# yamoling/lle

Measured on AMD Instinct MI355X. Metric: env-steps/s (agents x envs x steps/s), level-6 batch 65536, higher is better.
Workload: dtype u8

## Files before the change

lle_amd/csrc/obs_stream.hpp:

```cpp
#pragma once
#include <hip/hip_runtime.h>
#include <stdint.h>

#include <type_traits>

#include "tables.h"

namespace lle {

__device__ __forceinline__ void wave_sync() {
    __builtin_amdgcn_fence(__ATOMIC_RELEASE, "wavefront");
    __builtin_amdgcn_wave_barrier();
    __builtin_amdgcn_fence(__ATOMIC_ACQUIRE, "wavefront");
}

__device__ __forceinline__ uint32_t xcd_block(uint32_t b, uint32_t n_blocks) {
    const uint32_t x = b & 7u, q = n_blocks >> 3, r = n_blocks & 7u;
    return x * q + (x < r ? x : r) + (b >> 3);
}
__device__ __forceinline__ uint32_t xcd_block_dir(uint32_t b, uint32_t n_blocks, uint32_t flags) {
    const uint32_t blk = xcd_block(b, n_blocks);
    return (flags & LAUNCH_REVERSE) ? n_blocks - 1u - blk : blk;
}

__device__ __forceinline__ uint32_t row_rotation(uint32_t wave_id, uint32_t rows_per_wave, int64_t n_here, uint32_t flags) {
    const uint32_t r = wave_id & (rows_per_wave - 1u);
    return ((flags & LAUNCH_ROTATE_ROWS) && (int64_t)r < n_here && n_here == (int64_t)rows_per_wave) ? r : 0u;
}
__device__ __forceinline__ uint32_t rotated(uint32_t k, uint32_t rot, uint32_t n) {
    const uint32_t kk = k + rot;
    return kk >= n ? kk - n : kk;
}

typedef uint32_t u32x4 __attribute__((ext_vector_type(4)));
#define LLE_COPY_ROWS(SRC)                                                                                              \
    for (uint32_t r0 = wave_in_wg; r0 < rows; r0 += 8 * waves_per_wg) {                                                \
        const uint32_t r1 = r0 + waves_per_wg, r2 = r1 + waves_per_wg, r3 = r2 + waves_per_wg, r4 = r3 + waves_per_wg, \
                       r5 = r4 + waves_per_wg, r6 = r5 + waves_per_wg, r7 = r6 + waves_per_wg;                          \
        const u32x4 z = {0, 0, 0, 0};                                                                                   \
        u32x4 v0 = SRC(r0), v1 = z, v2 = z, v3 = z, v4 = z, v5 = z, v6 = z, v7 = z;                                      \
        if (r1 < rows) v1 = SRC(r1);                                                                                    \
        if (r2 < rows) v2 = SRC(r2);                                                                                    \
        if (r3 < rows) v3 = SRC(r3);                                                                                    \
        if (r4 < rows) {                                                                                                \
            v4 = SRC(r4);                                                                                               \
            if (r5 < rows) v5 = SRC(r5);                                                                                \
            if (r6 < rows) v6 = SRC(r6);                                                                                \
            if (r7 < rows) v7 = SRC(r7);                                                                                \
        }                                                                                                               \
        __builtin_amdgcn_sched_barrier(0);                        \
        dst[r0 * 64] = v0;                                                                                              \
        if (r1 < rows) dst[r1 * 64] = v1;                                                                               \
        if (r2 < rows) dst[r2 * 64] = v2;                                                                               \
        if (r3 < rows) dst[r3 * 64] = v3;                                                                               \
        if (r4 < rows) {                                                                                                \
            dst[r4 * 64] = v4;                                                                                          \
            if (r5 < rows) dst[r5 * 64] = v5;                                                                           \
            if (r6 < rows) dst[r6 * 64] = v6;                                                                           \
            if (r7 < rows) dst[r7 * 64] = v7;                                                                           \
        }                                                                                                               \
    }
__device__ __forceinline__ void copy_tables_to_lds(const uint8_t* __restrict__ tables, uint8_t* lds, uint32_t tab_bytes,
                                                   uint32_t lane, uint32_t wave_in_wg, uint32_t waves_per_wg) {
    const u32x4* __restrict__ src = reinterpret_cast<const u32x4*>(tables) + lane;
    u32x4* dst = reinterpret_cast<u32x4*>(lds) + lane;
    const uint32_t rows = tab_bytes / 1024;
#define LLE_SRC1(r) src[(r) * 64]
    LLE_COPY_ROWS(LLE_SRC1)
#undef LLE_SRC1
}

__device__ __forceinline__ void copy_tables2_to_lds(const uint8_t* __restrict__ t1, uint32_t bytes1, const uint8_t* __restrict__ t2, uint32_t bytes2,
                                                    uint8_t* lds, uint32_t lane, uint32_t wave_in_wg, uint32_t waves_per_wg) {
    const u32x4* __restrict__ s1 = reinterpret_cast<const u32x4*>(t1) + lane;
    const u32x4* __restrict__ s2 = reinterpret_cast<const u32x4*>(t2) + lane;
    u32x4* dst = reinterpret_cast<u32x4*>(lds) + lane;
    const uint32_t rows1 = bytes1 / 1024, rows = rows1 + bytes2 / 1024;
#define LLE_SRC2(r) (*((r) < rows1 ? s1 + (r) * 64 : s2 + ((r) - rows1) * 64))
    LLE_COPY_ROWS(LLE_SRC2)
#undef LLE_SRC2
}
#undef LLE_COPY_ROWS

__device__ __forceinline__ void expand_packed_tables(const uint8_t* __restrict__ pk, uint8_t* lds, uint32_t HW, uint32_t n_lay, uint32_t lds_meta, uint32_t lds_dyn,
                                                     uint32_t tail_bytes, uint32_t tid, uint32_t T) {
    const uint64_t* __restrict__ m4 = reinterpret_cast<const uint64_t*>(pk);
    const uint16_t* __restrict__ idx = reinterpret_cast<const uint16_t*>(pk + packed_meta_bytes(HW));
    const uint64_t* __restrict__ lay = reinterpret_cast<const uint64_t*>(pk + packed_meta_bytes(HW) + packed_idx_bytes(n_lay));
    const uint4* __restrict__ tail = reinterpret_cast<const uint4*>(pk + packed_meta_bytes(HW) + packed_idx_bytes(n_lay) + ((n_lay * 8u + 15u) & ~15u));
    const uint32_t n4 = (HW + 3u) / 4u, nt = tail_bytes / 16u;
    const uint64_t w0 = tid < n4 ? m4[tid] : 0ull;
    const uint32_t i0 = tid < n_lay ? (uint32_t)idx[tid] : 0u;
    const uint64_t l0 = tid < n_lay ? lay[tid] : 0ull;
    uint4 t0 = {0u, 0u, 0u, 0u};
    if (tid < nt) t0 = tail[tid];
    auto widen = [](uint64_t w) { return uint4{(uint32_t)w & 0xFFFFu, (uint32_t)(w >> 16) & 0xFFFFu, (uint32_t)(w >> 32) & 0xFFFFu, (uint32_t)(w >> 48)}; };
    uint4* z = reinterpret_cast<uint4*>(lds);
    for (uint32_t i = tid; i < lds_meta / 16u; i += T) z[i] = uint4{0u, 0u, 0u, 0u};
    uint4* md = reinterpret_cast<uint4*>(lds + lds_meta);
    if (tid < n4) md[tid] = widen(w0);
    for (uint32_t i = tid + T; i < n4; i += T) md[i] = widen(m4[i]);
    uint4* td = reinterpret_cast<uint4*>(lds + lds_dyn);
    if (tid < nt) td[tid] = t0;
    for (uint32_t i = tid + T; i < nt; i += T) td[i] = tail[i];
    asm volatile("s_waitcnt lgkmcnt(0)\n\ts_barrier" ::: "memory");
    uint64_t* ld = reinterpret_cast<uint64_t*>(lds);
    if (tid < n_lay) ld[i0] = l0;
    for (uint32_t i = tid + T; i < n_lay; i += T) ld[idx[i]] = lay[i];
}

__device__ __forceinline__ uint32_t mad24(uint32_t a, uint32_t b, uint32_t c) {
    uint32_t r;
    asm("v_mad_u32_u24 %0, %1, %2, %3" : "=v"(r) : "v"(a), "v"(b), "v"(c));
    return r;
}

template <typename T>
__device__ __forceinline__ void small_store(T* p, T v) {
#ifdef LLE_SMALL_WT
    if constexpr (sizeof(T) == 1) {
        asm volatile("global_store_byte %0, %1, off sc1" ::"v"(p), "v"((uint32_t)(uint8_t)v) : "memory");
    } else if constexpr (sizeof(T) == 2) {
        asm volatile("global_store_short %0, %1, off sc1" ::"v"(p), "v"((uint32_t)(uint16_t)v) : "memory");
    } else if constexpr (sizeof(T) == 4) {
        uint32_t w;
        __builtin_memcpy(&w, &v, 4);
        asm volatile("global_store_dword %0, %1, off sc1" ::"v"(p), "v"(w) : "memory");
    } else {
        static_assert(sizeof(T) == 8, "small_store: 1, 2, 4 or 8 bytes");
        uint64_t w;
        __builtin_memcpy(&w, &v, 8);
        asm volatile("global_store_dwordx2 %0, %1, off sc1" ::"v"(p), "v"(w) : "memory");
    }
#else
    *p = v;
#endif
}

template <bool WT>
__device__ __forceinline__ void stream_store(uint4* p, const uint4& v) {
    if constexpr (WT) {
        const u32x4 w = {v.x, v.y, v.z, v.w};
        asm volatile("global_store_dwordx4 %0, %1, off sc1\n\ts_nop 1" ::"v"(p), "v"(w));
    } else {
        *p = v;
    }
}

template <bool WT>
__device__ __forceinline__ void stream_row(uint4* __restrict__ dst, const uint4* srcv, uint32_t first, uint32_t n_chunks, uint32_t lane) {
    uint32_t c = first + lane;
    for (; c + 192u < n_chunks; c += 256u) {
        const uint4 q0 = srcv[c], q1 = srcv[c + 64u], q2 = srcv[c + 128u], q3 = srcv[c + 192u];
        stream_store<WT>(dst + c, q0);
        stream_store<WT>(dst + c + 64u, q1);
        stream_store<WT>(dst + c + 128u, q2);
        stream_store<WT>(dst + c + 192u, q3);
    }
    for (; c < n_chunks; c += 64u) stream_store<WT>(dst + c, srcv[c]);
}

template <bool WT>
__device__ __forceinline__ void stream_whole_row(uint4* __restrict__ dst, const uint4* srcv, uint32_t n_chunks, uint32_t lane) {
    const uint32_t c0 = lane, c1 = lane + 64u;
    const uint4 v0 = srcv[c0 < n_chunks ? c0 : 0u], v1 = srcv[c1 < n_chunks ? c1 : 0u];
    if (c0 < n_chunks) stream_store<WT>(dst + c0, v0);
    if (c1 < n_chunks) stream_store<WT>(dst + c1, v1);
    if (n_chunks > 128u) stream_row<WT>(dst, srcv, 128u, n_chunks, lane);
}

template <bool WT>
__device__ __forceinline__ void stream_row_tail(uint4* __restrict__ dst, const uint4* srcv, uint32_t n_chunks, uint32_t head_lo, uint32_t head_n,
                                                uint32_t lane, uint32_t head2_lo = 0, uint32_t head2_n = 0) {
    const uint32_t n_tail = n_chunks - head_n - head2_n;
    auto chunk_of = [&](uint32_t i) {
        uint32_t c = i + (i >= head_lo ? head_n : 0u);
        if (head2_n) c += c >= head2_lo ? head2_n : 0u;
        return c;
    };
    const uint32_t i0 = lane, i1 = lane + 64u;
    const uint32_t c0 = chunk_of(i0), c1 = chunk_of(i1);
    const uint4 v0 = srcv[i0 < n_tail ? c0 : 0u], v1 = srcv[i1 < n_tail ? c1 : 0u];
    if (i0 < n_tail) stream_store<WT>(dst + c0, v0);
    if (i1 < n_tail) stream_store<WT>(dst + c1, v1);
    for (uint32_t i = lane + 128u; i < n_tail; i += 64u) {
        const uint32_t c = chunk_of(i);
        stream_store<WT>(dst + c, srcv[c]);
    }
}

template <bool WT>
__device__ __forceinline__ void stream_row_dyn(uint4* __restrict__ dst, const uint4* srcv, const uint16_t* tab, uint32_t n_dyn, uint32_t c0, uint32_t c1,
                                               uint32_t lane) {
    const uint4 v0 = srcv[c0 != 0xFFFFu ? c0 : 0u], v1 = srcv[c1 != 0xFFFFu ? c1 : 0u];
    if (c0 != 0xFFFFu) stream_store<WT>(dst + c0, v0);
    if (c1 != 0xFFFFu) stream_store<WT>(dst + c1, v1);
    for (uint32_t i = lane + 128u; i < n_dyn; i += 64u) {
        const uint32_t c = tab[i];
        stream_store<WT>(dst + c, srcv[c]);
    }
}

__device__ __forceinline__ uint4 widen_chunk16(const int8_t* tmpl, uint32_t q, uint32_t one, uint32_t sel_lo, uint32_t sel_hi) {
    const uint2 w = reinterpret_cast<const uint2*>(tmpl)[q];
    uint32_t o[4];
#pragma unroll
    for (int k = 0; k < 4; k++) {
        const uint32_t src = k < 2 ? w.x : w.y;
        const uint32_t x = __builtin_amdgcn_perm(src, src, (k & 1) ? sel_hi : sel_lo);
        o[k] = __umul24(x & 0x00010001u, one) | ((x & 0x00800080u) << 8);
    }
    return make_uint4(o[0], o[1], o[2], o[3]);
}
__device__ __forceinline__ uint4 widen_chunk32(const int8_t* tmpl, uint32_t q) {
    const uint32_t w = reinterpret_cast<const uint32_t*>(tmpl)[q];
    uint32_t o[4];
#pragma unroll
    for (int k = 0; k < 4; k++) {
        const uint32_t b = (w >> (8 * k)) & 0xFFu;
        o[k] = ((b & 1u) ? 0x3F800000u : 0u) | ((b & 0x80u) << 24);
    }
    return make_uint4(o[0], o[1], o[2], o[3]);
}
struct WideConsts { uint32_t one, sel_lo, sel_hi, sh, lane; };
__device__ __forceinline__ WideConsts wide_consts(uint32_t et, uint32_t lane) {
    uint32_t z = 0;
    asm volatile("" : "+s"(z));
    asm volatile("" : "+v"(lane));
    WideConsts c;
    c.one = (et == OBS_F16 ? 0x3C00u : 0x3F80u) | z;
    c.sel_lo = 0x0c010c00u | z;
    c.sel_hi = 0x0c030c02u | z;
    c.sh = obs_elem_shift(et) + z;
    c.lane = lane;
    return c;
}
template <bool WT>
__device__ __forceinline__ void stream_wide(uint4* __restrict__ dst, const int8_t* tmpl, uint32_t n_chunks, uint32_t et, uint32_t lane_in) {
    const WideConsts c = wide_consts(et, lane_in);
    const uint32_t n_out = n_chunks << c.sh;
    if (c.sh == 2u) {
#pragma clang loop unroll(disable)
        for (uint32_t q = c.lane; q < n_out; q += 64u) stream_store<WT>(dst + q, widen_chunk32(tmpl, q));
    } else {
#pragma clang loop unroll(disable)
        for (uint32_t q = c.lane; q < n_out; q += 64u) stream_store<WT>(dst + q, widen_chunk16(tmpl, q, c.one, c.sel_lo, c.sel_hi));
    }
}
template <bool WT>
__device__ __forceinline__ void stream_wide_dyn(uint4* __restrict__ dst, const int8_t* tmpl, const uint16_t* tab, uint32_t t_lo, uint32_t t_hi, uint32_t c_base,
                                                uint32_t et, uint32_t lane_in) {
    const WideConsts c = wide_consts(et, lane_in);
#pragma clang loop unroll(disable)
    for (uint32_t i = (t_lo << c.sh) + c.lane; i < (t_hi << c.sh); i += 64u) {
        const uint32_t q = (((uint32_t)tab[i >> c.sh] - c_base) << c.sh) + (i & ((1u << c.sh) - 1u));
        stream_store<WT>(dst + q, c.sh == 2u ? widen_chunk32(tmpl, q) : widen_chunk16(tmpl, q, c.one, c.sel_lo, c.sel_hi));
    }
}

template <bool WT>
__device__ __forceinline__ void store_heads(int8_t* __restrict__ obs, uint64_t obs_stride, int64_t env0, int64_t n_here, uint32_t head_lo,
                                            uint32_t head_n, const uint4& v, uint32_t lane, uint32_t rot = 0, uint32_t head2_lo = 0, uint32_t head2_n = 0) {
    const uint32_t chunk = lane < head_n ? head_lo + lane : head2_lo + (lane - head_n);
    if (lane < head_n + head2_n)
        for (uint32_t k = 0; k < (uint32_t)n_here; k++)
            stream_store<WT>(reinterpret_cast<uint4*>(obs + (uint64_t)(env0 + rotated(k, rot, (uint32_t)n_here)) * obs_stride) + chunk, v);
}

template <bool CAN_WIDE, typename F>
__device__ __forceinline__ void dispatch_stream(uint32_t lflags, F&& f) {
    const bool wt = (lflags & LAUNCH_WRITE_THROUGH) != 0;
    if constexpr (CAN_WIDE) {
        if (lflags & LAUNCH_OBS_ELEM_MASK) {
            if (wt) f(std::true_type{}, std::true_type{});
            else f(std::false_type{}, std::true_type{});
            return;
        }
    }
    if (wt) f(std::true_type{}, std::false_type{});
    else f(std::false_type{}, std::false_type{});
}

template <bool WT, bool HEAD = false, bool INCR = false, bool WIDE = false>
__device__ __forceinline__ void write_observations(int A, int L, uint32_t D, uint32_t n_chunks, uint64_t obs_stride,
                                                   const uint64_t* dyn, int8_t* tmpl, const uint32_t* scratch,
                                                   uint32_t scr_stride, int8_t* __restrict__ obs, int64_t env0,
                                                   int64_t n_here, uint32_t lane, uint32_t head_lo = 0, uint32_t head_n = 0, uint32_t rot = 0,
                                                   const uint16_t* dyn_chunks = nullptr, uint32_t n_dyn_chunks = 0, uint32_t et = OBS_I8) {
    static_assert(!(WIDE && HEAD), "the kernels with row heads carry no widening code: the launcher never sends them a widened launch");
    uint32_t dc0 = 0xFFFFu, dc1 = 0xFFFFu;
    if constexpr (INCR) {
        dc0 = lane < n_dyn_chunks ? (uint32_t)dyn_chunks[lane] : 0xFFFFu;
        dc1 = lane + 64u < n_dyn_chunks ? (uint32_t)dyn_chunks[lane + 64u] : 0xFFFFu;
    }
    const bool has_d0 = lane < D;
    const uint64_t e0 = has_d0 ? dyn[lane] : 0ull;
    const uint32_t d0_idx = dyn_index(e0);
    const int32_t d0_base = dyn_base(e0);
    const uint32_t d0_refs = dyn_refs(e0), d0_gem = dyn_gem(e0);
    const uint32_t d0_r0 = dyn_ref0(e0), d0_r1 = dyn_ref1(e0);
    const uint32_t d0_w0 = d0_refs >= 1 ? 1u + ref_word(d0_r0) : 0u, d0_s0 = d0_refs >= 1 ? ref_bit(d0_r0) : 0u;
    const uint32_t d0_w1 = d0_refs >= 2 ? 1u + ref_word(d0_r1) : 0u, d0_s1 = d0_refs >= 2 ? ref_bit(d0_r1) : 0u;
    const uint32_t d0_wg = d0_gem != NO_GEM ? (uint32_t)L + 1u : 0u, d0_sg = d0_gem != NO_GEM ? gem_bit(d0_gem) : 0u;
    const bool is_agent_lane = (int)lane < A;
    const uint4* srcv = reinterpret_cast<const uint4*>(tmpl);

    for (uint32_t k0 = 0; k0 < (uint32_t)n_here; k0++) {
        const uint32_t k = rotated(k0, rot, (uint32_t)n_here);
        const uint32_t* sc = scratch + k * scr_stride;
        {
            const uint32_t lit = ((sc[d0_w0] >> d0_s0) | (sc[d0_w1] >> d0_s1) | (sc[d0_wg] >> d0_sg)) & 1u;
            if (has_d0) tmpl[d0_idx] = (int8_t)(lit ? 1 : d0_base);
        }
        for (uint32_t d = lane + 64u; d < D; d += 64) {
            const uint64_t e = dyn[d];
            const uint32_t refs = dyn_refs(e), gem = dyn_gem(e);
            const uint32_t r0 = dyn_ref0(e), r1 = dyn_ref1(e);
            const uint32_t w0 = refs >= 1 ? 1u + ref_word(r0) : 0u, w1 = refs >= 2 ? 1u + ref_word(r1) : 0u;
            const uint32_t wg = gem != NO_GEM ? (uint32_t)L + 1u : 0u;
            const uint32_t lit = ((sc[w0] >> (refs >= 1 ? ref_bit(r0) : 0u)) | (sc[w1] >> (refs >= 2 ? ref_bit(r1) : 0u)) |
                                  (sc[wg] >> (gem != NO_GEM ? gem_bit(gem) : 0u))) & 1u;
            tmpl[dyn_index(e)] = (int8_t)(lit ? 1 : dyn_base(e));
        }
        const uint32_t agent_idx = is_agent_lane ? sc[L + 2 + lane] : 0u;
        if (is_agent_lane) tmpl[agent_idx] = 1;
        wave_sync();
        uint4* __restrict__ dst = reinterpret_cast<uint4*>(obs + (uint64_t)(env0 + k) * obs_stride);
        if constexpr (WIDE) {
            if constexpr (INCR) stream_wide_dyn<WT>(dst, tmpl, dyn_chunks, 0u, n_dyn_chunks, 0u, et, lane);
            else stream_wide<WT>(dst, tmpl, n_chunks, et, lane);
        } else if constexpr (INCR) stream_row_dyn<WT>(dst, srcv, dyn_chunks, n_dyn_chunks, dc0, dc1, lane);
        else if constexpr (HEAD) stream_row_tail<WT>(dst, srcv, n_chunks, head_lo, head_n, lane);
        else stream_whole_row<WT>(dst, srcv, n_chunks, lane);
        wave_sync();
        if (is_agent_lane) tmpl[agent_idx] = 0;
    }
}

template <bool WT, bool INCR = false, bool WIDE = false>
__device__ __forceinline__ void write_observations_split(int A, int L, uint32_t D, uint32_t lo, uint32_t hi, uint64_t obs_stride,
                                                         const uint64_t* dyn, int8_t* tmpl, const uint32_t* records,
                                                         uint32_t scr_stride, int8_t* __restrict__ obs, int64_t wg_env0,
                                                         int64_t n_wg_here, uint32_t lane, const uint16_t* dyn_chunks = nullptr, uint32_t n_dyn_chunks = 0,
                                                         uint32_t et = OBS_I8) {
    const uint32_t b_lo = lo * 16u, b_hi = hi * 16u;
    uint32_t t_lo = 0, t_hi = 0;
    if constexpr (INCR) {
        for (uint32_t i = lane; i < ((n_dyn_chunks + 63u) & ~63u); i += 64) {
            const uint32_t c = i < n_dyn_chunks ? (uint32_t)dyn_chunks[i] : 0xFFFFFFFFu;
            t_lo += (uint32_t)__popcll(__ballot(c < lo));
            t_hi += (uint32_t)__popcll(__ballot(c < hi));
        }
    }
    uint32_t d_lo = 0, d_hi = 0;
    for (uint32_t d = lane; d < ((D + 63u) & ~63u); d += 64) {
        const uint32_t idx = d < D ? dyn_index(dyn[d]) : 0xFFFFFFFFu;
        d_lo += (uint32_t)__popcll(__ballot(idx < b_lo));
        d_hi += (uint32_t)__popcll(__ballot(idx < b_hi));
    }
    const bool has_d0 = d_lo + lane < d_hi;
    const uint64_t e0 = has_d0 ? dyn[d_lo + lane] : 0ull;
    const uint32_t d0_idx = has_d0 ? dyn_index(e0) - b_lo : 0u;
    const int32_t d0_base = dyn_base(e0);
    const uint32_t d0_refs = dyn_refs(e0), d0_gem = dyn_gem(e0);
    const uint32_t d0_r0 = dyn_ref0(e0), d0_r1 = dyn_ref1(e0);
    const uint32_t d0_w0 = d0_refs >= 1 ? 1u + ref_word(d0_r0) : 0u, d0_s0 = d0_refs >= 1 ? ref_bit(d0_r0) : 0u;
    const uint32_t d0_w1 = d0_refs >= 2 ? 1u + ref_word(d0_r1) : 0u, d0_s1 = d0_refs >= 2 ? ref_bit(d0_r1) : 0u;
    const uint32_t d0_wg = d0_gem != NO_GEM ? (uint32_t)L + 1u : 0u, d0_sg = d0_gem != NO_GEM ? gem_bit(d0_gem) : 0u;
    const bool is_agent_lane = (int)lane < A;
    const uint4* srcv = reinterpret_cast<const uint4*>(tmpl);
    const uint32_t n_mine = hi - lo;

    for (int64_t k = 0; k < n_wg_here; k++) {
        const uint32_t* sc = records + (uint32_t)k * scr_stride;
        {
            const uint32_t lit = ((sc[d0_w0] >> d0_s0) | (sc[d0_w1] >> d0_s1) | (sc[d0_wg] >> d0_sg)) & 1u;
            if (has_d0) tmpl[d0_idx] = (int8_t)(lit ? 1 : d0_base);
        }
        for (uint32_t d = d_lo + lane + 64u; d < d_hi; d += 64) {
            const uint64_t e = dyn[d];
            const uint32_t refs = dyn_refs(e), gem = dyn_gem(e);
            const uint32_t r0 = dyn_ref0(e), r1 = dyn_ref1(e);
            const uint32_t w0 = refs >= 1 ? 1u + ref_word(r0) : 0u, w1 = refs >= 2 ? 1u + ref_word(r1) : 0u;
            const uint32_t wg = gem != NO_GEM ? (uint32_t)L + 1u : 0u;
            const uint32_t lit = ((sc[w0] >> (refs >= 1 ? ref_bit(r0) : 0u)) | (sc[w1] >> (refs >= 2 ? ref_bit(r1) : 0u)) |
                                  (sc[wg] >> (gem != NO_GEM ? gem_bit(gem) : 0u))) & 1u;
            tmpl[dyn_index(e) - b_lo] = (int8_t)(lit ? 1 : dyn_base(e));
        }
        const uint32_t agent_idx = is_agent_lane ? sc[L + 2 + lane] : 0xFFFFFFFFu;
        const bool agent_here = agent_idx >= b_lo && agent_idx < b_hi;
        if (agent_here) tmpl[agent_idx - b_lo] = 1;
        wave_sync();
        uint4* __restrict__ dst = reinterpret_cast<uint4*>(obs + (uint64_t)(wg_env0 + k) * obs_stride) + ((uint64_t)lo << (WIDE ? obs_elem_shift(et) : 0u));
        if constexpr (WIDE) {
            if constexpr (INCR) stream_wide_dyn<WT>(dst, tmpl, dyn_chunks, t_lo, t_hi, lo, et, lane);
            else stream_wide<WT>(dst, tmpl, n_mine, et, lane);
        } else if constexpr (INCR) {
            for (uint32_t i = t_lo + lane; i < t_hi; i += 64u) {
                const uint32_t c = (uint32_t)dyn_chunks[i] - lo;
                stream_store<WT>(dst + c, srcv[c]);
            }
        } else {
            stream_whole_row<WT>(dst, srcv, n_mine, lane);
        }
        wave_sync();
        if (agent_here) tmpl[agent_idx - b_lo] = 0;
    }
}

__device__ __forceinline__ void elem_eval(uint32_t e, const uint32_t* sc, int A, int L, uint32_t HW, const uint8_t* laser_layer,
                                          uint32_t gem_layer, uint32_t& idx, int32_t& val, bool& on) {
    const uint32_t cell = elem_cell(e), i5 = elem_index(e), off = elem_bit(e), type = elem_type(e);
    const uint32_t colour = (sc[L + 2 + A + (i5 >> 2)] >> ((i5 & 3u) * 8u)) & 0xFFu;
    const bool is_gem = type == ELEM_GEM;
    const uint32_t llayer = laser_layer ? (uint32_t)laser_layer[colour] : (uint32_t)A + colour;
    idx = (is_gem ? gem_layer : llayer) * HW + cell;
    val = type == ELEM_SOURCE ? -1 : 1;
    on = type == ELEM_SOURCE ? true : (is_gem ? ((sc[L + 1] >> i5) & 1u) != 0 : ((sc[1 + i5] >> off) & 1u) != 0);
}
template <bool WT, bool HEAD = false, bool INCR = false, bool WIDE = false>
__device__ __forceinline__ void write_observations_env(int A, int L, uint32_t HW, uint32_t n_elems, uint32_t n_chunks,
                                                       uint64_t obs_stride, const uint32_t* elems, const int8_t* bare,
                                                       int8_t* tmpl, const uint32_t* scratch, uint32_t scr_stride,
                                                       int8_t* __restrict__ obs, int64_t env0, int64_t n_here, uint32_t lane,
                                                       const uint8_t* laser_layer = nullptr, uint32_t gem_layer_in = 0xFFFFFFFFu,
                                                       uint32_t head_lo = 0, uint32_t head_n = 0, uint32_t rot = 0,
                                                       const uint16_t* dyn_chunks = nullptr, uint32_t n_dyn_chunks = 0, uint32_t head2_lo = 0, uint32_t head2_n = 0,
                                                       uint32_t et = OBS_I8) {
    static_assert(!(WIDE && HEAD), "no widening in the kernels with row heads");
    uint32_t dc0 = 0xFFFFu, dc1 = 0xFFFFu;
    if constexpr (INCR) {
        dc0 = lane < n_dyn_chunks ? (uint32_t)dyn_chunks[lane] : 0xFFFFu;
        dc1 = lane + 64u < n_dyn_chunks ? (uint32_t)dyn_chunks[lane + 64u] : 0xFFFFu;
    }
    const uint32_t gem_layer = gem_layer_in == 0xFFFFFFFFu ? (uint32_t)(2 * A + 2) : gem_layer_in;
    const bool has_e0 = lane < n_elems;
    const uint32_t e0 = has_e0 ? elems[lane] : 0u;
    const uint32_t e0_cell = elem_cell(e0), e0_i5 = elem_index(e0), e0_off = elem_bit(e0), e0_type = elem_type(e0);
    const bool e0_gem = e0_type == ELEM_GEM, e0_src = e0_type == ELEM_SOURCE;
    const uint32_t e0_colw = (uint32_t)(L + 2 + A) + (e0_i5 >> 2), e0_colsh = (e0_i5 & 3u) * 8u;
    const uint32_t e0_onw = e0_gem ? (uint32_t)L + 1u : (e0_src ? 0u : 1u + e0_i5);
    const uint32_t e0_onsh = e0_gem ? e0_i5 : e0_off;
    const int8_t e0_val = e0_src ? (int8_t)-1 : (int8_t)1;
    const uint32_t e0_base = (e0_gem ? gem_layer : (uint32_t)A) * HW + e0_cell, e0_mul = (e0_gem || laser_layer) ? 0u : HW;
    const uint32_t e0_always = (has_e0 && e0_src) ? 1u : 0u, e0_dyn = (has_e0 && !e0_src) ? 1u : 0u;
    const bool is_agent_lane = (int)lane < A;
    const uint4* srcv = reinterpret_cast<const uint4*>(tmpl);
    for (uint32_t k0 = 0; k0 < (uint32_t)n_here; k0++) {
        const uint32_t k = rotated(k0, rot, (uint32_t)n_here);
        const uint32_t* sc = scratch + k * scr_stride;
        const uint32_t colour = (sc[e0_colw] >> e0_colsh) & 0xFFu, onw = sc[e0_onw];
        uint32_t idx0 = e0_base + __umul24(colour, e0_mul);
        if (laser_layer && !e0_gem) idx0 = (uint32_t)laser_layer[colour] * HW + e0_cell;
        const bool on0 = ((e0_always | (e0_dyn & (onw >> e0_onsh))) & 1u) != 0u;
        if (on0) tmpl[idx0] = e0_val;
        for (uint32_t d = lane + 64u; d < n_elems; d += 64) {
            uint32_t idx; int32_t val; bool on;
            elem_eval(elems[d], sc, A, L, HW, laser_layer, gem_layer, idx, val, on);
            if (on) tmpl[idx] = (int8_t)val;
        }
        const uint32_t agent_idx = is_agent_lane ? sc[L + 2 + lane] : 0u;
        if (is_agent_lane) tmpl[agent_idx] = 1;
        wave_sync();
        uint4* __restrict__ dst = reinterpret_cast<uint4*>(obs + (uint64_t)(env0 + k) * obs_stride);
        if constexpr (WIDE) {
            if constexpr (INCR) stream_wide_dyn<WT>(dst, tmpl, dyn_chunks, 0u, n_dyn_chunks, 0u, et, lane);
            else stream_wide<WT>(dst, tmpl, n_chunks, et, lane);
        } else if constexpr (INCR) stream_row_dyn<WT>(dst, srcv, dyn_chunks, n_dyn_chunks, dc0, dc1, lane);
        else if constexpr (HEAD) stream_row_tail<WT>(dst, srcv, n_chunks, head_lo, head_n, lane, head2_lo, head2_n);
        else stream_whole_row<WT>(dst, srcv, n_chunks, lane);
        wave_sync();
        if (on0) {
            int8_t back = 0;
            if (!e0_gem && colour >= (uint32_t)A) back = bare[idx0];
            tmpl[idx0] = back;
        }
        for (uint32_t d = lane + 64u; d < n_elems; d += 64) {
            uint32_t idx; int32_t val; bool on;
            elem_eval(elems[d], sc, A, L, HW, laser_layer, gem_layer, idx, val, on);
            if (on) tmpl[idx] = bare[idx];
        }
        if (is_agent_lane) tmpl[agent_idx] = 0;
    }
}

}
```

lle_amd/csrc/step_kernel.hpp:

```cpp
#pragma once
#include "kernel_common.hpp"
#include "partial_stream.hpp"
#include "step_lanes.hpp"

namespace lle {


__device__ __forceinline__ EnvOutputs load_uniform(const EnvOutputs* p) {
    static_assert(sizeof(EnvOutputs) == 64, "one s_load_dwordx16");
    typedef uint32_t u32x16 __attribute__((ext_vector_type(16)));
    u32x16 w;
    asm volatile("s_load_dwordx16 %0, %1, 0x0\n\ts_waitcnt lgkmcnt(0)" : "=s"(w) : "s"(p) : "memory");
    EnvOutputs o;
    __builtin_memcpy(&o, &w, sizeof o);
    return o;
}

constexpr size_t KERNARG_ENV_OUT = ((sizeof(BatchPtrs) + alignof(LaunchArgs) - 1) / alignof(LaunchArgs)) * alignof(LaunchArgs) + offsetof(LaunchArgs, out);
__device__ __forceinline__ const EnvOutputs* kernarg_env_out() {
    return reinterpret_cast<const EnvOutputs*>((const char*)__builtin_amdgcn_kernarg_segment_ptr() + KERNARG_ENV_OUT);
}

template <int G, int LM, int MODE, bool ML1, int LX = -1>
__global__ void __launch_bounds__(256, (G >= 8 ? 3 : 4)) step_kernel(BatchPtrs P, LaunchArgs K) {
    constexpr bool PARTIAL = MODE == 9;
    constexpr bool GEN = (MODE >= 2 && MODE <= 5) || MODE == 7 || MODE == 8 || PARTIAL, ROLL = MODE >= 1 && MODE <= 3;
    constexpr bool PES = MODE == 3 || MODE == 5 || MODE == 8;
    constexpr bool BM = LM >= 8;
    constexpr int LR = BM ? 1 : LM;
    constexpr bool CAN_SPLIT = G >= 8 && !PES && !PARTIAL;
    constexpr bool HEAD = MODE == 6 || MODE == 7 || MODE == 8;
    const bool split = CAN_SPLIT && (K.flags & LAUNCH_SPLIT_ROWS) != 0;
#ifdef LLE_STAMP_SINGLE
    constexpr bool STAMPED = true;
#else
    constexpr bool STAMPED = ROLL;
#endif
    uint64_t* const stamps = STAMPED ? K.stamps : nullptr;
#undef LLE_STAMP
#define LLE_STAMP(i)                                                                              \
    do {                                                                                          \
        if (STAMPED && stamps && lane == 0) stamps[(uint64_t)wave_id * 8 + (i)] = __builtin_amdgcn_s_memrealtime(); \
    } while (0)
    const uint32_t EPW = K.envs_per_wave < (uint32_t)(64 / G) ? K.envs_per_wave : (uint32_t)(64 / G);
    constexpr int NW = (2 * G + 7) / 8;
    extern __shared__ __attribute__((aligned(16))) uint8_t lds[];
    const uint32_t lane = threadIdx.x & 63u, wave_in_wg = threadIdx.x >> 6, waves_per_wg = blockDim.x >> 6;
    const uint32_t blk = xcd_block_dir(blockIdx.x, gridDim.x, K.flags);
    const uint32_t wave_id = blk * waves_per_wg + wave_in_wg;
    const uint8_t* __restrict__ tables = P.tables;
    const InitRecord* __restrict__ initp = P.init;
    uint32_t map_idx = 0u;
    if (GEN) {
        const uint32_t EPW0 = K.envs_per_wave < (uint32_t)(64 / G) ? K.envs_per_wave : (uint32_t)(64 / G);
        map_idx = map_index_of(K, K.env_base + (int64_t)(blk * waves_per_wg) * EPW0);
        tables += (uint64_t)map_idx * K.table_stride;
        initp += map_idx;
    }
    const MapHeader* __restrict__ hdr = reinterpret_cast<const MapHeader*>(tables);
    const int A = (int)hdr->A, L = LX >= 0 ? LX : (int)hdr->L, W = (int)hdr->W;
    const uint32_t a = lane & (G - 1), grp = lane / G;
    const int64_t As = agent_stride_of(A, L);
    const int64_t env0 = K.env_base + (int64_t)wave_id * EPW;
    const int64_t env = env0 + grp;
    const bool env_ok = grp < EPW && env < K.env_limit;
    const bool me = env_ok && (int)a < A;
    const bool write_obs = !PARTIAL && hdr->obs_supported && !(K.flags & STEP_NO_OBS);
    const uint32_t h_HW = hdr->HW, h_obs_stride = hdr->obs_stride, h_n_chunks = hdr->n_chunks, h_D = hdr->D;
#define LLE_ET() (HEAD ? (uint32_t)OBS_I8 : (K.flags & LAUNCH_OBS_ELEM_MASK) >> LAUNCH_OBS_ELEM_SHIFT)
#define LLE_PITCH() ((uint64_t)h_obs_stride << obs_elem_shift(LLE_ET()))
    uint32_t h_beam_full[LR];
#pragma unroll
    for (int b = 0; b < LR; b++) h_beam_full[b] = (!BM && b < L) ? hdr->beam_full[b] : 0u;
    const uint32_t h_enabled = hdr->enabled_mask;
    const uint32_t h_chain = BM ? hdr->chain_mask : 0u;
    const uint32_t h_off_cell_meta = hdr->off_cell_meta, h_off_dyn = hdr->off_dyn, h_off_template = hdr->off_template;
    const uint32_t h_max_layers = ML1 ? 1u : hdr->max_layers;
    constexpr bool CAN_INCR = !ROLL && !PARTIAL && !HEAD;
    const uint32_t h_off_dyn_chunks = CAN_INCR ? (PES ? hdr->off_pes_dyn_chunks : hdr->off_dyn_chunks) : 0u;
    const uint32_t h_n_dyn_chunks = CAN_INCR ? (PES ? hdr->n_pes_dyn_chunks : hdr->n_dyn_chunks) : 0u;
    const bool incr = CAN_INCR && (K.flags & STEP_INCREMENTAL_OBS) != 0 && h_n_dyn_chunks < h_n_chunks;
    const uint32_t h_off_recolour = PES ? hdr->off_recolour : 0u, h_off_bare = PES ? hdr->off_bare : 0u;
    const uint32_t h_off_elems = PES ? hdr->off_elems : 0u, h_n_elems = PES ? hdr->n_elems : 0u;
    constexpr bool ENV_OUT = MODE == 4 || MODE == 5 || MODE == 7 || MODE == 8 || PARTIAL;
    EnvOutputs O_early = {};
    uint32_t h_G = 0, h_H = 0;
    constexpr bool EARLY_OUT = MODE == 7;
    if (EARLY_OUT && K.env_out) O_early = K.out;
    if (ENV_OUT) { h_G = hdr->G; h_H = hdr->H; }
    uint32_t h_init_beams[LR];
#pragma unroll
    for (int b = 0; b < LR; b++) h_init_beams[b] = (!BM && b < L) ? initp->beams[b] : 0u;
    const int64_t n_here = (K.env_limit - env0) < (int64_t)EPW ? (K.env_limit - env0) : (int64_t)EPW;
    const uint32_t amask = (1u << A) - 1u;
#define LLE_ROT() ((ROLL && PES) ? 0u : row_rotation(wave_id, EPW, n_here, K.flags))
    LLE_STAMP(0);

    uint32_t pos = 0xFFFF0000u + a, avail = 0, beams[LR];
    uint64_t raw_bits = 0;
    uint32_t gems = 0;
#pragma unroll
    for (int b = 0; b < LR; b++) beams[b] = 0;
    const int64_t env_c = env_ok ? env : 0;
    uint64_t* const p_bits = P.bits + env_c;
    uint32_t* const p_gems = P.gems + env_c;
    uint32_t* const p_beams = P.beams + env_c * L;
    uint16_t* const p_pos = P.pos + env_c * As + a;
    uint8_t* const p_avail = P.avail + env_c * As + a;
    uint8_t* const p_err = P.err + env_c;
    uint8_t* const p_evcount = P.evcount + env_c;
    uint8_t* const p_events = P.events + env_c * 2 * As;
    uint8_t* const p_done = P.done + env_c;
#define LLE_LATE(field, offset) ((GEN || ROLL) ? P.field + (offset) : p_##field)
#define LLE_ENV_LATE(name)                                   \
    int64_t name = env_c;                                    \
    if ((GEN || ROLL) && !HEAD) asm volatile("" : "+v"(name))
    uint32_t init_pos_a = 0xFFFF0000u + a, init_avail_a = 0;
    uint64_t init_bits = 0;
    uint32_t init_gems = 0;
    constexpr int CWM = LM / 4;
    const int CW = src_stride_of(L) / 4;
    uint32_t colw[CWM], env_enabled = h_enabled;
    constexpr bool PRE_BEAMS = PES && !ROLL && LM <= 8;
    const bool shared_init = PES && !ROLL && hdr->recolour_exact != 0u;
    uint32_t env_init_beams[LR];
#pragma unroll
    for (int b = 0; b < LR; b++) env_init_beams[b] = 0u;
#pragma unroll
    for (int q = 0; q < CWM; q++) colw[q] = 0;
    uint32_t act_given = 4u;
    constexpr int BPL = (HEAD && BM) ? (LM + G - 1) / G : 1;
    uint32_t bm_pre[BPL];
#pragma unroll
    for (int k = 0; k < BPL; k++) bm_pre[k] = 0u;
    constexpr bool PRE_STATS = (MODE == 0 || MODE == 6 || MODE == 7 || MODE == 8) && LM <= 8;
    int64_t stats_old = 0;
#define LLE_LOAD_STATE() \
    do { \
        if (env_ok) { \
            raw_bits = *p_bits; \
            gems = *p_gems; \
        _Pragma("unroll") \
            for (int b = 0; b < LR; b++) \
                if (!BM && b < L) beams[b] = p_beams[b]; \
        } \
        if (me) { \
            pos = (uint32_t)*p_pos; \
            avail = (uint32_t)*p_avail; \
            init_pos_a = (PES && !shared_init) ? (uint32_t)P.init_pos[env * As + a] : (uint32_t)initp->pos[a]; \
            init_avail_a = (PES && !shared_init) ? (uint32_t)P.init_avail[env * As + a] : (uint32_t)initp->avail[a]; \
            if (!ROLL && !(K.flags & STEP_SAMPLE_ACTIONS)) \
                act_given = K.actions_in ? (uint32_t)K.actions_in[env * A + a] : (uint32_t)P.actions[env * As + a]; \
        } \
        if (HEAD && BM && env_ok) { \
        _Pragma("unroll") \
            for (int k = 0; k < BPL; k++) \
                if ((int)a + k * G < L) bm_pre[k] = p_beams[(int)a + k * G]; \
        } \
        init_bits = initp->bits; \
        init_gems = initp->gems; \
        if (PRE_STATS) stats_old = stats_preload(P.stats, wave_id, lane); \
        if (PES && env_ok) { \
            env_enabled = P.src_enabled[env]; \
        _Pragma("unroll") \
            for (int q = 0; q < CWM; q++) \
                if (q < CW) colw[q] = reinterpret_cast<const uint32_t*>(P.src_colour)[env * CW + q]; \
            if ((K.flags & STEP_AUTO_RESET) && !shared_init) { \
                init_bits = P.init_bits[env]; \
                init_gems = P.init_gems[env]; \
        _Pragma("unroll") \
                for (int b = 0; b < LR; b++) \
                    if (PRE_BEAMS && b < L) env_init_beams[b] = P.init_beams[env * L + b]; \
            } \
        } \
    } while (0)

    const uint32_t head_lo = HEAD ? (PES ? hdr->pes_head_lo : hdr->head_lo) : 0u;
    const uint32_t head_n = (HEAD && write_obs && !split && !incr) ? (PES ? hdr->pes_head_n : hdr->head_n) : 0u;
    const uint32_t head2_lo = (HEAD && PES) ? hdr->pes_head2_lo : 0u, head2_n = (HEAD && PES && head_n) ? hdr->pes_head2_n : 0u;
    uint4 head_v = {0u, 0u, 0u, 0u};
    if (HEAD) {
        if (lane < head_n + head2_n)
            head_v = reinterpret_cast<const uint4*>(tables + (PES ? h_off_bare : h_off_template))[lane < head_n ? head_lo + lane : head2_lo + (lane - head_n)];
        LLE_LOAD_STATE();
    }
    uint32_t bt_full = 0u, bt_init = 0u;
    if (BM && (int)threadIdx.x < L) {
        bt_full = hdr->beam_full[threadIdx.x];
        bt_init = initp->beams[threadIdx.x];
    }
    const uint32_t tab_off = hdr->off_cell_lay;
    const uint32_t tab_cells = ((hdr->off_dyn - tab_off) + 1023u) & ~1023u;
    const uint32_t tab_bytes = PARTIAL ? (tab_cells < hdr->lds_table_bytes ? tab_cells : hdr->lds_table_bytes)
                                       : (split ? hdr->lds_split_table_bytes : hdr->lds_table_bytes);
    const bool use_sets = PARTIAL && K.win_sets != nullptr;
    const uint32_t ext_bytes = PES ? hdr->ext_bytes : (use_sets ? win_sets_bytes(hdr->HW) : 0u);
    constexpr int PB = CAN_SPLIT ? 8 : 1;
    const uint32_t cpw = (h_n_chunks + waves_per_wg - 1u) / waves_per_wg;
    const uint32_t c_lo = wave_in_wg * cpw < h_n_chunks ? wave_in_wg * cpw : h_n_chunks;
    const uint32_t c_hi = c_lo + cpw < h_n_chunks ? c_lo + cpw : h_n_chunks;
    uint32_t pre_bits[PB];
    uint32_t pre_neg = 0xFFFFFFFFu;
#pragma unroll
    for (int q = 0; q < PB; q++) pre_bits[q] = 0u;
    if (CAN_SPLIT && split) {
        const uint16_t* __restrict__ bits = reinterpret_cast<const uint16_t*>(tables + sizeof(MapHeader)) + c_lo;
#pragma unroll
        for (int q = 0; q < PB; q++)
            if (lane + 64u * q < c_hi - c_lo) pre_bits[q] = bits[lane + 64u * q];
        if (lane < TMPL_NEG_MAX) pre_neg = reinterpret_cast<const uint32_t*>(tables + sizeof(MapHeader) + tmpl_bits_bytes(h_n_chunks))[lane];
        if (!HEAD) LLE_LOAD_STATE();
    }
    if (PES) copy_tables2_to_lds(tables + tab_off, tab_bytes, tables + h_off_bare, ext_bytes, lds, lane, wave_in_wg, waves_per_wg);
    else if (use_sets) copy_tables2_to_lds(tables + tab_off, tab_bytes, K.win_sets + (uint64_t)map_idx * win_table_bytes(hdr->HW), ext_bytes, lds, lane, wave_in_wg, waves_per_wg);
    else if (CAN_SPLIT && GEN && split && (K.flags & LAUNCH_PACKED_TABLES))
        expand_packed_tables(tables + hdr->off_packed, lds, h_HW, hdr->packed_n_lay, h_off_cell_meta - tab_off, h_off_dyn - tab_off, h_off_template - h_off_dyn,
                             threadIdx.x, blockDim.x);
    else copy_tables_to_lds(tables + tab_off, lds, tab_bytes, lane, wave_in_wg, waves_per_wg);
    constexpr uint32_t bt_bytes = BM ? 2u * LM * 4u : 0u;
    uint32_t* beam_tab = reinterpret_cast<uint32_t*>(lds + tab_bytes + ext_bytes);
    if (BM && (int)threadIdx.x < L) {
        beam_tab[threadIdx.x] = bt_full;
        beam_tab[LM + threadIdx.x] = bt_init;
    }
    const uint32_t pm_bytes = PARTIAL ? (use_sets ? 0u : partial_bitmap_bytes(hdr->H, (uint32_t)W)) + 32u : 0u;
    uint32_t* const part_bm = reinterpret_cast<uint32_t*>(lds + tab_bytes + ext_bytes + bt_bytes);
    uint8_t* const part_col = lds + tab_bytes + ext_bytes + bt_bytes + (pm_bytes - 32u);
    if (PARTIAL) {
        for (uint32_t w = threadIdx.x; w < (pm_bytes - 32u) / 4u; w += blockDim.x) part_bm[w] = 0u;
        if ((int)threadIdx.x < L) part_col[threadIdx.x] = hdr->beam_colour[threadIdx.x];
    }
    LLE_STAMP(7);
    if (HEAD) {
        __builtin_amdgcn_s_waitcnt(0x0F70);
        const uint32_t hgroup = MODE != 6 ? 1u : ((K.flags & LAUNCH_HEAD_GROUP4) ? 4u : ((K.flags & LAUNCH_HEAD_GROUP2) ? 2u : 1u));
        if (hgroup == 1u) {
            if (head_n && n_here > 0) {
                if (K.flags & LAUNCH_WRITE_THROUGH) store_heads<true>(P.obs, h_obs_stride, env0, n_here, head_lo, head_n, head_v, lane, LLE_ROT(), head2_lo, head2_n);
                else store_heads<false>(P.obs, h_obs_stride, env0, n_here, head_lo, head_n, head_v, lane, LLE_ROT(), head2_lo, head2_n);
            }
            asm volatile("s_waitcnt lgkmcnt(0)\n\ts_barrier" ::: "memory");
        } else {
            asm volatile("s_waitcnt lgkmcnt(0)\n\ts_barrier" ::: "memory");
            if (head_n && (wave_in_wg & (hgroup - 1u)) == 0u) {
                for (uint32_t q = 0; q < hgroup && wave_in_wg + q < waves_per_wg; q++) {
                    const int64_t e0q = env0 + (int64_t)q * EPW;
                    int64_t nq = K.env_limit - e0q;
                    nq = nq < 0 ? 0 : (nq > (int64_t)EPW ? (int64_t)EPW : nq);
                    if (nq > 0) {
                        if (K.flags & LAUNCH_WRITE_THROUGH) store_heads<true>(P.obs, h_obs_stride, e0q, nq, head_lo, head_n, head_v, lane);
                        else store_heads<false>(P.obs, h_obs_stride, e0q, nq, head_lo, head_n, head_v, lane);
                    }
                }
            }
        }
    } else {
        __syncthreads();
        if (!(CAN_SPLIT && split)) LLE_LOAD_STATE();
    }

    const uint64_t* cell_lay = reinterpret_cast<const uint64_t*>(lds);
    const uint32_t* cell_meta = reinterpret_cast<const uint32_t*>(lds + (h_off_cell_meta - tab_off));
    const uint64_t* dyn = reinterpret_cast<const uint64_t*>(lds + (h_off_dyn - tab_off));
    const uint16_t* dyn_chunks = PES ? reinterpret_cast<const uint16_t*>(lds + tab_bytes + (h_off_dyn_chunks - h_off_bare))
                                     : reinterpret_cast<const uint16_t*>(lds + (h_off_dyn_chunks - tab_off));
    const uint32_t scr_stride = (uint32_t)(L + A + 2 + (PES ? CW : 0)) | 1u;
    const uint32_t part_pitch = PARTIAL ? (((uint32_t)(A * (2 * A + 3)) * K.partial_k * K.partial_k + 15u) & ~15u) : 0u;
    const uint32_t row_area = PARTIAL ? K.partial_E * part_pitch + 16u : h_obs_stride;
    const uint32_t priv_bytes = row_area + (PARTIAL ? ((EPW * scr_stride * 4u + 15u) & ~15u) : 64u * scr_stride * 4u) + (PES ? PES_WAVE_EXTRA_BYTES : 0u);
    int8_t* tmpl = reinterpret_cast<int8_t*>(lds + tab_bytes + ext_bytes + bt_bytes + pm_bytes + wave_in_wg * priv_bytes);
    uint32_t* scratch = reinterpret_cast<uint32_t*>(tmpl + row_area);
    const int8_t* bare = reinterpret_cast<const int8_t*>(lds + tab_bytes);
    const uint32_t* elems = reinterpret_cast<const uint32_t*>(lds + tab_bytes + (h_off_elems - h_off_bare));
    if (split) {
        tmpl = reinterpret_cast<int8_t*>(lds + tab_bytes + bt_bytes + wave_in_wg * cpw * 16u);
        scratch = reinterpret_cast<uint32_t*>(lds + tab_bytes + bt_bytes + waves_per_wg * cpw * 16u) + wave_in_wg * EPW * scr_stride;
        uint4* mine = reinterpret_cast<uint4*>(tmpl);
        if (hdr->off_tmpl_bits) {
            auto expand = [](uint32_t b) {
                return uint4{((b & 15u) * 0x00204081u) & 0x01010101u, (((b >> 4) & 15u) * 0x00204081u) & 0x01010101u,
                             (((b >> 8) & 15u) * 0x00204081u) & 0x01010101u, ((b >> 12) * 0x00204081u) & 0x01010101u};
            };
#pragma unroll
            for (int q = 0; q < PB; q++)
                if (lane + 64u * q < c_hi - c_lo) mine[lane + 64u * q] = expand(pre_bits[q]);
            const uint16_t* __restrict__ bits = reinterpret_cast<const uint16_t*>(tables + sizeof(MapHeader)) + c_lo;
            for (uint32_t c = lane + 64u * PB; c < c_hi - c_lo; c += 64) mine[c] = expand(bits[c]);
            if (lane < hdr->tmpl_neg_n && pre_neg >= c_lo * 16u && pre_neg < c_hi * 16u) tmpl[pre_neg - c_lo * 16u] = (int8_t)-1;
        } else {
            const uint4* __restrict__ pristine = reinterpret_cast<const uint4*>(tables + h_off_template) + c_lo;
            for (uint32_t c = lane; c < c_hi - c_lo; c += 64) mine[c] = pristine[c];
        }
    } else if (PARTIAL) {
        if (!use_sets) partial_bitmap_fill(part_bm, cell_lay, cell_meta, (int)hdr->H, W);
    } else {
        const uint4* pristine = PES ? reinterpret_cast<const uint4*>(bare) : reinterpret_cast<const uint4*>(lds + (h_off_template - tab_off));
        uint4* mine = reinterpret_cast<uint4*>(tmpl);
        for (uint32_t c = lane; c < h_n_chunks; c += 64) mine[c] = pristine[c];
    }
    uint32_t* const bm = scratch + grp * scr_stride + 1;
    if (HEAD && BM) {
        if (env_ok) {
#pragma unroll
            for (int k = 0; k < BPL; k++)
                if ((int)a + k * G < L) bm[(int)a + k * G] = bm_pre[k];
        }
    } else if (BM && env_ok) {
        for (int b = (int)a; b < L; b += G) bm[b] = p_beams[b];
    }
    wave_sync();
    if (!HEAD) __builtin_amdgcn_s_waitcnt(0x0F70);
    LLE_STAMP(1);

    uint32_t alive = (uint32_t)raw_bits & 0xFFFFu, arrived = (uint32_t)(raw_bits >> 16) & 0xFFFFu, occ = (uint32_t)(raw_bits >> 32) & 0xFFFFu;
    uint32_t ghost = (uint32_t)(raw_bits >> GHOST_SHIFT);
    const uint32_t enabled = PES ? env_enabled : h_enabled, max_layers = h_max_layers;
    LLE_STAMP(2);

    StepCounts cnt = {0, 0, 0, 0, 0, 0, 0};
    constexpr bool CNT_LDS = ROLL && PES && G >= 2;
    uint32_t* const cnt_lds = scratch + 64u * scr_stride + grp * 8u;
    if (CNT_LDS && env_ok && a == 0) {
#pragma unroll
        for (int q = 0; q < 7; q++) cnt_lds[q] = 0u;
    }
    const uint32_t n_steps = ROLL ? (K.n_steps ? K.n_steps : 1u) : 1u;
    for (uint32_t it = 0; it < n_steps; it++) {
    const uint64_t t_now = K.t + it;
    uint8_t* __restrict__ actions_out = P.actions;
    uint32_t* __restrict__ reward_out = P.reward;
    int8_t* __restrict__ obs_out = P.obs;
    if (ROLL && K.ring_slots) {
        uint32_t slot = (uint32_t)K.ring_pos + it;
        while (slot >= K.ring_slots) slot -= K.ring_slots;
        actions_out = K.ring_actions + (int64_t)slot * K.ring_env_count * As;
        reward_out = K.ring_reward + (int64_t)slot * K.ring_env_count;
        obs_out = K.ring_obs + (int64_t)slot * K.ring_env_count * (int64_t)LLE_PITCH();
    }

    uint32_t was_reset = 0;
    if (K.flags & STEP_AUTO_RESET) {
        const bool over = env_ok && ((alive | ghost) != amask || arrived == amask);
        pos = (over && me) ? init_pos_a : pos;
        avail = (over && me) ? init_avail_a : avail;
        alive = over ? ((uint32_t)init_bits & 0xFFFFu) : alive;
        arrived = over ? ((uint32_t)(init_bits >> 16) & 0xFFFFu) : arrived;
        occ = over ? ((uint32_t)(init_bits >> 32) & 0xFFFFu) : occ;
        ghost = over ? 0u : ghost;
        gems = over ? init_gems : gems;
#pragma unroll
        for (int b = 0; b < LR; b++)
            if (!BM && b < L && !(PES && shared_init))
                beams[b] = over ? (PES ? (PRE_BEAMS ? env_init_beams[b] : P.init_beams[env_ok ? env * L + b : 0]) : h_init_beams[b]) : beams[b];
        if (BM && over && !(PES && shared_init))
            for (int b = (int)a; b < L; b += G) bm[b] = PES ? P.init_beams[env * L + b] : beam_tab[LM + b];
        if (PES && shared_init && __ballot(over) != 0ull) {
            const uint32_t* rtab0 = reinterpret_cast<const uint32_t*>(lds + tab_bytes + (h_off_recolour - h_off_bare));
            if (!BM) {
#pragma unroll
                for (int b = 0; b < LR; b++)
                    if (b < L) {
                        const uint32_t c = (colw[b >> 2] >> ((b & 3) * 8)) & 0xFFu;
                        const uint32_t m = ((env_enabled >> b) & 1u) ? rtab0[b * (A + 1) + 1 + (int)(c < (uint32_t)A ? c : 0u)] : 0u;
                        beams[b] = over ? m : beams[b];
                    }
            } else if (over) {
                for (int b = (int)a; b < L; b += G) {
                    const uint32_t c = (colw[b >> 2] >> ((b & 3) * 8)) & 0xFFu;
                    bm[b] = ((env_enabled >> b) & 1u) ? rtab0[b * (A + 1) + 1 + (int)(c < (uint32_t)A ? c : 0u)] : 0u;
                }
            }
        }
        was_reset = over ? 1u : 0u;
        if (PES && !ROLL && (K.flags & STEP_RECOLOUR_RESETS) && __ballot(over) != 0ull) {
            const uint32_t* rtab = reinterpret_cast<const uint32_t*>(lds + tab_bytes + (h_off_recolour - h_off_bare));
            const uint64_t rkey = action_step_key(K.seed ^ RECOLOUR_SALT, t_now);
#pragma unroll
            for (int b = 0; b < LM; b++) {
                if (b < L) {
                    const uint32_t* row = rtab + b * (A + 1);
                    const uint32_t ok = row[0] & amask;
                    const uint32_t field = action_field(action_hash_pair(rkey, (uint64_t)(K.env_offset + env), (uint32_t)b >> 1), (uint32_t)b);
                    const uint32_t k = (field * (uint32_t)__popc(ok)) >> 16;
                    const bool mine = ((ok >> a) & 1u) != 0u && (uint32_t)__popc(ok & ((1u << a) - 1u)) == k;
                    const uint32_t pick = grp_or<G>(mine ? a + 1u : 0u);
                    const uint32_t sh = (uint32_t)(b & 3) * 8u, old_c = (colw[b >> 2] >> sh) & 0xFFu;
                    const uint32_t c = (over && pick) ? pick - 1u : old_c;
                    colw[b >> 2] = (colw[b >> 2] & ~(0xFFu << sh)) | (c << sh);
                    if (over && a == 0) P.init_beams[env * L + b] = ((env_enabled >> b) & 1u) ? row[1u + (c < (uint32_t)A ? c : 0u)] : 0u;
                }
            }
            if (over && a == 0) {
#pragma unroll
                for (int q = 0; q < CWM; q++)
                    if (q < CW) reinterpret_cast<uint32_t*>(P.src_colour)[env * CW + q] = colw[q];
            }
        }
    }

    uint32_t act = 4u;
    if (K.flags & STEP_SAMPLE_ACTIONS) {
        const uint32_t hp = action_hash_pair(action_step_key(K.seed, t_now), (uint64_t)(K.env_offset + env), a >> 1);
        act = sample_action(avail, action_field(hp, a));
        if (me) small_store(&actions_out[env * As + a], (uint8_t)act);
    } else if (!ROLL) {
        act = act_given;
        if (me && K.actions_in) P.actions[env * As + a] = (uint8_t)act;
    } else if (K.actions_in) {
        if (me) {
            act = (uint32_t)K.actions_in[env * A + a];
            P.actions[env * As + a] = (uint8_t)act;
        }
    } else if (me) {
        act = (uint32_t)actions_out[env * As + a];
    }

    uint64_t evw[NW];
    uint32_t n_ev, meta_step, err;
    bool stepped;
    step_lanes<G, LR, ML1, PES, CWM, true, BM>(cell_lay, cell_meta, A, L, W, max_layers, h_beam_full, a, me, env_ok, enabled, colw, act, pos, avail,
                                               alive, arrived, occ, gems, beams, err, evw, n_ev, meta_step, stepped, nullptr, bm, beam_tab, h_chain);
    LLE_STAMP(3);

    auto post_step = [&]() {
    LLE_ENV_LATE(env_p);
    if (stepped) avail_lanes<G>(a, me, pos, occ, alive, arrived, meta_step, avail);
#pragma unroll
    for (int k = 0; k < NW; k++) evw[k] = grp_or64<G>(evw[k]);
    if (env_ok && a == 0) {
        small_store(LLE_LATE(err, env_p), (uint8_t)err);
        small_store(LLE_LATE(evcount, env_p), (uint8_t)(n_ev | (was_reset << 7)));
        {
            uint8_t* row = LLE_LATE(events, env_p * 2 * As);
            if (G >= 2) {
                uint32_t* __restrict__ w = reinterpret_cast<uint32_t*>(row);
#pragma unroll
                for (int k = 0; k < G / 2; k++) small_store(&w[k], (uint32_t)(evw[k >> 1] >> ((k & 1) * 32)));
            } else {
                small_store(reinterpret_cast<uint16_t*>(row), (uint16_t)evw[0]);
            }
        }
        small_store(LLE_LATE(done, env_p), (uint8_t)(((alive | ghost) != amask || arrived == amask) ? 1 : 0));
        uint32_t n_died = 0, n_gem = 0;
#pragma unroll
        for (int k = 0; k < NW; k++) {
            n_died += (uint32_t)__popcll(evw[k] & 0x2020202020202020ull);
            n_gem += (uint32_t)__popcll(evw[k] & 0x1010101010101010ull);
        }
        const uint32_t n_exit = n_ev - n_died - n_gem;
        const uint32_t bonus = (err == 0 && arrived == amask) ? 1u : 0u;
        small_store(&reward_out[env], n_gem | (n_exit << 8) | (n_died << 16) | (bonus << 24));
        if (CNT_LDS) {
            const uint32_t add[7] = {1u, n_gem, n_exit, n_died, err != 0 ? 1u : 0u, was_reset, bonus};
#pragma unroll
            for (int q = 0; q < 7; q++) __hip_atomic_fetch_add(&cnt_lds[q], add[q], __ATOMIC_RELAXED, __HIP_MEMORY_SCOPE_WAVEFRONT);
        } else {
            cnt.steps += 1u; cnt.gems += n_gem; cnt.exits += n_exit; cnt.died += n_died;
            cnt.invalid += err != 0 ? 1u : 0u; cnt.resets += was_reset; cnt.bonus += bonus;
        }
    }
    if (ENV_OUT && K.env_out) {
        const EnvOutputs O = EARLY_OUT ? O_early : load_uniform(kernarg_env_out());
        const int n_gems = (int)h_G, len = 3 * A + n_gems;
        if (me) {
            const int64_t ia = env * A + a;
            if (O.alive) small_store(&O.alive[ia], (uint8_t)((alive >> a) & 1u));
            if (O.arrived) small_store(&O.arrived[ia], (uint8_t)((arrived >> a) & 1u));
            if (O.available) {
                uint8_t* o = O.available + ia * 5;
#pragma unroll
                for (int k = 0; k < 5; k++) small_store(&o[k], (uint8_t)((avail >> k) & 1u));
            }
        }
#define LLE_STATE_IJ()                                               \
    float fi = (float)(pos & 0xFFu), fj = (float)(pos >> 8);         \
    if (O.normalize_state) {                                         \
        fi = (float)((double)(pos & 0xFFu) / (double)h_H);           \
        fj = (float)((double)(pos >> 8) / (double)W);                \
    }
        if (HEAD) {
            const uint32_t st_off = (EPW * scr_stride * 4u + 15u) & ~15u;
            const bool staged = !split && O.state && (len & 3) == 0 && (reinterpret_cast<uintptr_t>(O.state) & 15u) == 0u &&
                                st_off + EPW * (uint32_t)len * 4u <= 64u * scr_stride * 4u;
            if (O.state) {
                float* st = staged ? reinterpret_cast<float*>(reinterpret_cast<uint8_t*>(scratch) + st_off) + grp * (uint32_t)len : O.state + env * len;
                if (me) {
                    LLE_STATE_IJ()
                    st[2 * a] = fi;
                    st[2 * a + 1] = fj;
                    st[2 * A + n_gems + (int)a] = ((alive >> a) & 1u) ? 1.0f : 0.0f;
                }
                if (env_ok)
                    for (int g = (int)a; g < n_gems; g += G) st[2 * A + g] = ((gems >> g) & 1u) ? 1.0f : 0.0f;
                if (staged) {
                    wave_sync();
                    const float4* src4 = reinterpret_cast<const float4*>(reinterpret_cast<uint8_t*>(scratch) + st_off);
                    float4* dst4 = reinterpret_cast<float4*>(O.state + env0 * len);
                    const uint32_t n4 = n_here > 0 ? (uint32_t)n_here * (uint32_t)len / 4u : 0u;
                    for (uint32_t c = lane; c < n4; c += 64u) dst4[c] = src4[c];
                    wave_sync();
                }
            }
        } else {
            if (me && O.state) {
                float* st = O.state + env * len;
                LLE_STATE_IJ()
                small_store(&st[2 * a], fi);
                small_store(&st[2 * a + 1], fj);
                small_store(&st[2 * A + n_gems + (int)a], ((alive >> a) & 1u) ? 1.0f : 0.0f);
            }
            if (env_ok && O.state)
                for (int g = (int)a; g < n_gems; g += G) small_store(&O.state[env * len + 2 * A + g], ((gems >> g) & 1u) ? 1.0f : 0.0f);
        }
#undef LLE_STATE_IJ
        if (env_ok && a == 0) {
            if (O.done) small_store(&O.done[env], (uint8_t)(((alive | ghost) != amask || arrived == amask) ? 1 : 0));
            if (O.reward) {
                uint32_t n_died = 0, n_gem = 0;
#pragma unroll
                for (int k = 0; k < NW; k++) {
                    n_died += (uint32_t)__popcll(evw[k] & 0x2020202020202020ull);
                    n_gem += (uint32_t)__popcll(evw[k] & 0x1010101010101010ull);
                }
                const float gem = (float)n_gem, died = (float)n_died, ex = (float)(n_ev - n_died - n_gem);
                const float bonus = (err == 0 && arrived == amask) ? 1.0f : 0.0f;
                if (O.reward_kind == 0) {
                    small_store(&O.reward[env], gem + ex - died + bonus);
                } else {
                    const bool dead = n_died > 0;
                    float* o = O.reward + env * 4;
                    small_store(&o[0], dead ? 0.f : gem); small_store(&o[1], dead ? 0.f : ex); small_store(&o[2], -died); small_store(&o[3], dead ? 0.f : bonus);
                }
            }
        }
    }
    };

    if (env_ok && a == 0) {
        uint32_t* sc = scratch + grp * scr_stride;
        sc[0] = 0u;
#pragma unroll
        for (int b = 0; b < LR; b++)
            if (!BM && b < L) sc[1 + b] = beams[b];
        sc[L + 1] = ~gems;
        if (PES) {
#pragma unroll
            for (int q = 0; q < CWM; q++)
                if (q < CW) sc[L + 2 + A + q] = colw[q];
        }
    }
    if (me) scratch[grp * scr_stride + L + 2 + a] = PARTIAL ? pos : a * h_HW + cell_of(pos, W);
    if (split) {
        asm volatile("s_waitcnt lgkmcnt(0)\n\ts_barrier" ::: "memory");
    } else {
        wave_sync();
    }
    LLE_STAMP(4);
    const bool post_first = ROLL || PARTIAL || (K.flags & LAUNCH_POST_FIRST) || (!(K.flags & LAUNCH_POST_LAST) && blockIdx.x * 4u >= gridDim.x * 3u);
    if (post_first) post_step();

    const uint32_t et = LLE_ET();
    if (split) {
        if (write_obs) {
            const int64_t wg_env0 = K.env_base + (int64_t)(blk * waves_per_wg) * EPW;
            int64_t n_wg = K.env_limit - wg_env0;
            n_wg = n_wg < 0 ? 0 : (n_wg > (int64_t)(waves_per_wg * EPW) ? (int64_t)(waves_per_wg * EPW) : n_wg);
            const uint32_t* records = reinterpret_cast<const uint32_t*>(lds + tab_bytes + bt_bytes + waves_per_wg * cpw * 16u);
            dispatch_stream<!HEAD>(K.flags, [&](auto wt_, auto wide_) {
                constexpr bool WT = decltype(wt_)::value, WIDE = decltype(wide_)::value;
                if (CAN_INCR && incr) write_observations_split<WT, true, WIDE>(A, L, h_D, c_lo, c_hi, LLE_PITCH(), dyn, tmpl, records, scr_stride, obs_out, wg_env0, n_wg, lane, dyn_chunks, h_n_dyn_chunks, et);
                else write_observations_split<WT, false, WIDE>(A, L, h_D, c_lo, c_hi, LLE_PITCH(), dyn, tmpl, records, scr_stride, obs_out, wg_env0, n_wg, lane, nullptr, 0u, et);
            });
        }
        if (ROLL && n_steps > 1) asm volatile("s_waitcnt lgkmcnt(0)\n\ts_barrier" ::: "memory");
    } else if (PARTIAL) {
        asm volatile("s_waitcnt lgkmcnt(0)\n\ts_barrier" ::: "memory");
        const EnvOutputs O = load_uniform(kernarg_env_out());
        if (O.partial && n_here > 0)
            write_partial<true>(A, L, W, (int)K.partial_k, part_pitch, K.partial_E, h_max_layers, cell_lay, cell_meta, part_bm, part_col, tmpl, scratch,
                                scr_stride, O.partial, env0, n_here, lane, use_sets ? reinterpret_cast<const uint64_t*>(lds + tab_bytes) : nullptr, et);
    } else if (write_obs && n_here > 0) {
        dispatch_stream<!HEAD>(K.flags, [&](auto wt_, auto wide_) {
            constexpr bool WT = decltype(wt_)::value, WIDE = decltype(wide_)::value;
            if (PES && CAN_INCR && incr)
                write_observations_env<WT, false, true, WIDE>(A, L, h_HW, h_n_elems, h_n_chunks, LLE_PITCH(), elems, bare, tmpl, scratch, scr_stride, obs_out, env0, n_here,
                                                              lane, nullptr, 0xFFFFFFFFu, 0u, 0u, LLE_ROT(), dyn_chunks, h_n_dyn_chunks, 0u, 0u, et);
            else if (PES)
                write_observations_env<WT, HEAD, false, WIDE>(A, L, h_HW, h_n_elems, h_n_chunks, LLE_PITCH(), elems, bare, tmpl, scratch, scr_stride, obs_out, env0, n_here,
                                                              lane, nullptr, 0xFFFFFFFFu, head_lo, head_n, LLE_ROT(), nullptr, 0u, head2_lo, head2_n, et);
            else if (CAN_INCR && incr)
                write_observations<WT, false, true, WIDE>(A, L, h_D, h_n_chunks, LLE_PITCH(), dyn, tmpl, scratch, scr_stride, obs_out, env0, n_here, lane, 0u, 0u, LLE_ROT(),
                                                          dyn_chunks, h_n_dyn_chunks, et);
            else
                write_observations<WT, HEAD, false, WIDE>(A, L, h_D, h_n_chunks, LLE_PITCH(), dyn, tmpl, scratch, scr_stride, obs_out, env0, n_here, lane, head_lo, head_n,
                                                          LLE_ROT(), nullptr, 0u, et);
        });
    }
    wave_sync();
    if (!post_first) post_step();
    }
    LLE_STAMP(5);

    LLE_ENV_LATE(env_f);
    if (me) {
        small_store(LLE_LATE(pos, env_f * As + a), (uint16_t)pos);
        small_store(LLE_LATE(avail, env_f * As + a), (uint8_t)avail);
    }
    if (env_ok && a == 0) {
        small_store(LLE_LATE(bits, env_f), (uint64_t)alive | ((uint64_t)arrived << 16) | ((uint64_t)occ << 32) | ((uint64_t)ghost << GHOST_SHIFT));
        small_store(LLE_LATE(gems, env_f), gems);
        uint32_t* const beams_out = LLE_LATE(beams, env_f * L);
#pragma unroll
        for (int b = 0; b < LR; b++)
            if (!BM && b < L) small_store(&beams_out[b], beams[b]);
    }
    if (BM && env_ok) {
        uint32_t* const beams_out = LLE_LATE(beams, env_f * L);
        for (int b = (int)a; b < L; b += G) small_store(&beams_out[b], bm[b]);
#undef LLE_LATE
#undef LLE_ENV_LATE
#undef LLE_LOAD_STATE
#undef LLE_ROT
#undef LLE_ET
#undef LLE_PITCH
    }
    if (CNT_LDS && env_ok && a == 0) {
        cnt.steps = cnt_lds[0]; cnt.gems = cnt_lds[1]; cnt.exits = cnt_lds[2]; cnt.died = cnt_lds[3];
        cnt.invalid = cnt_lds[4]; cnt.resets = cnt_lds[5]; cnt.bonus = cnt_lds[6];
    }
    flush_stats(P.stats, wave_id, cnt, A, lane, PRE_STATS, stats_old);
    if (STAMPED && stamps) {
        asm volatile("s_waitcnt vmcnt(0)" ::: "memory");
        LLE_STAMP(6);
    }
}

template <int G, int LM, int MODE, bool ML1, int LX = -1>
static hipError_t launch_step_glp(const BatchPtrs& P, const LaunchArgs& K, uint32_t n_waves, uint32_t wpw, uint32_t lds, hipStream_t stream) {
    static std::atomic<uint32_t> noted{0};
    const uint32_t note_bit = (K.flags & LAUNCH_DRY_RUN) ? 2u : 1u;
    if (!(noted.load(std::memory_order_relaxed) & note_bit)) {
        noted.fetch_or(note_bit, std::memory_order_relaxed);
        debug_note(debug_key(DBG_STEP, G, LM, MODE, ML1, LX), (K.flags & LAUNCH_DRY_RUN) != 0);
    }
    if (K.flags & LAUNCH_DRY_RUN) return hipSuccess;
    dim3 grid((n_waves + wpw - 1) / wpw), block(64 * wpw);
    if (lds > 64 * 1024) {
        static LdsGrant granted;
        hipError_t e = granted.ensure(reinterpret_cast<const void*>(&step_kernel<G, LM, MODE, ML1, LX>), lds);
        if (e != hipSuccess) return e;
    }
    hipLaunchKernelGGL((step_kernel<G, LM, MODE, ML1, LX>), grid, block, lds, stream, P, K);
    return hipGetLastError();
}
template <int MODE, int G, int LM>
static hipError_t launch_step_mode_gl(const BatchPtrs& P, const LaunchArgs& K, uint32_t n_waves, uint32_t wpw, uint32_t lds, hipStream_t stream) {
    const bool ml1 = (K.flags & LAUNCH_SINGLE_LAYER) != 0;
    if constexpr (LM == 4) {
        if (ml1) {
#define LLE_STEP_LX(X) case X: return launch_step_glp<G, 4, MODE, true, X>(P, K, n_waves, wpw, lds, stream);
            switch (K.n_sources) { LLE_STEP_LX(0) LLE_STEP_LX(1) LLE_STEP_LX(2) LLE_STEP_LX(3) LLE_STEP_LX(4) default: return hipErrorInvalidValue; }
#undef LLE_STEP_LX
        }
        return launch_step_glp<G, 4, MODE, false>(P, K, n_waves, wpw, lds, stream);
    } else {
        return ml1 ? launch_step_glp<G, LM, MODE, true>(P, K, n_waves, wpw, lds, stream)
                   : launch_step_glp<G, LM, MODE, false>(P, K, n_waves, wpw, lds, stream);
    }
}
template <int MODE, int G>
static hipError_t launch_step_mode_g(int lm, const BatchPtrs& P, const LaunchArgs& K, uint32_t n_waves, uint32_t wpw, uint32_t lds, hipStream_t stream) {
    if constexpr (MODE == 6 || MODE == 7 || MODE == 8 || MODE == 9) {
        if (lm == 4) return launch_step_mode_gl<MODE, G, 4>(P, K, n_waves, wpw, lds, stream);
        if (lm == 8) return launch_step_mode_gl<MODE, G, 8>(P, K, n_waves, wpw, lds, stream);
        return hipErrorInvalidValue;
    } else {
        switch (lm) {
            case 4: return launch_step_mode_gl<MODE, G, 4>(P, K, n_waves, wpw, lds, stream);
            case 8: return launch_step_mode_gl<MODE, G, 8>(P, K, n_waves, wpw, lds, stream);
            case 16: return launch_step_mode_gl<MODE, G, 16>(P, K, n_waves, wpw, lds, stream);
            default: return launch_step_mode_gl<MODE, G, 32>(P, K, n_waves, wpw, lds, stream);
        }
    }
}
template <int MODE>
static hipError_t launch_step_mode(int G, int lm, const BatchPtrs& P, const LaunchArgs& K, uint32_t n_waves, uint32_t wpw, uint32_t lds, hipStream_t stream) {
    switch (G) {
        case 1: return launch_step_mode_g<MODE, 1>(lm, P, K, n_waves, wpw, lds, stream);
        case 2: return launch_step_mode_g<MODE, 2>(lm, P, K, n_waves, wpw, lds, stream);
        case 4: return launch_step_mode_g<MODE, 4>(lm, P, K, n_waves, wpw, lds, stream);
        case 8: return launch_step_mode_g<MODE, 8>(lm, P, K, n_waves, wpw, lds, stream);
        default: return launch_step_mode_g<MODE, 16>(lm, P, K, n_waves, wpw, lds, stream);
    }
}

}
```

Before: 13.16 billion.

## Specialise HEAD kernels with uniform hot path and scalar-register pinning

For kernels with row heads, a hot path is added for the common write-through, no-rotation case. It streams observation rows with compile-time write-through and no rotation, and uses a simpler head-store loop. Uniform values are forced into SGPRs via readfirstlane and asm constraints, and some are parked in VGPRs across the step body to reduce scalar register pressure and recomputation. A runtime write-through cold path replaces the duplicated template instantiations, which risks extra branching and register-allocation side effects.

```diff
diff --git a/lle_amd/csrc/obs_stream.hpp b/lle_amd/csrc/obs_stream.hpp
--- a/lle_amd/csrc/obs_stream.hpp
+++ b/lle_amd/csrc/obs_stream.hpp
@@ -34,7 +34,9 @@
 
 typedef uint32_t u32x4 __attribute__((ext_vector_type(4)));
 #define LLE_COPY_ROWS(SRC)                                                                                              \
-    for (uint32_t r0 = wave_in_wg; r0 < rows; r0 += 8 * waves_per_wg) {                                                \
+    for (uint32_t rr = wave_in_wg; rr < rows; rr += 8 * waves_per_wg) {                                                \
+        uint32_t r0 = rr;                                                                                               \
+        if constexpr (UNI) asm volatile("" : "+s"(r0));                                                                 \
         const uint32_t r1 = r0 + waves_per_wg, r2 = r1 + waves_per_wg, r3 = r2 + waves_per_wg, r4 = r3 + waves_per_wg, \
                        r5 = r4 + waves_per_wg, r6 = r5 + waves_per_wg, r7 = r6 + waves_per_wg;                          \
         const u32x4 z = {0, 0, 0, 0};                                                                                   \
@@ -60,6 +62,7 @@
             if (r7 < rows) dst[r7 * 64] = v7;                                                                           \
         }                                                                                                               \
     }
+template <bool UNI = false>
 __device__ __forceinline__ void copy_tables_to_lds(const uint8_t* __restrict__ tables, uint8_t* lds, uint32_t tab_bytes,
                                                    uint32_t lane, uint32_t wave_in_wg, uint32_t waves_per_wg) {
     const u32x4* __restrict__ src = reinterpret_cast<const u32x4*>(tables) + lane;
@@ -70,6 +73,7 @@
 #undef LLE_SRC1
 }
 
+template <bool UNI = false>
 __device__ __forceinline__ void copy_tables2_to_lds(const uint8_t* __restrict__ t1, uint32_t bytes1, const uint8_t* __restrict__ t2, uint32_t bytes2,
                                                     uint8_t* lds, uint32_t lane, uint32_t wave_in_wg, uint32_t waves_per_wg) {
     const u32x4* __restrict__ s1 = reinterpret_cast<const u32x4*>(t1) + lane;
@@ -147,6 +151,11 @@
     }
 }
 
+__device__ __forceinline__ void stream_store_rt(uint4* p, const uint4& v, uint32_t wt) {
+    if (wt) stream_store<true>(p, v);
+    else stream_store<false>(p, v);
+}
+
 template <bool WT>
 __device__ __forceinline__ void stream_row(uint4* __restrict__ dst, const uint4* srcv, uint32_t first, uint32_t n_chunks, uint32_t lane) {
     uint32_t c = first + lane;
@@ -189,6 +198,17 @@
     }
 }
 
+__device__ __forceinline__ void stream_row_tail_rt(uint4* __restrict__ dst, const uint4* srcv, uint32_t n_chunks, uint32_t head_lo, uint32_t head_n,
+                                                   uint32_t lane, uint32_t wt, uint32_t head2_lo = 0, uint32_t head2_n = 0) {
+    const uint32_t n_tail = n_chunks - head_n - head2_n;
+#pragma clang loop unroll(disable)
+    for (uint32_t i = lane; i < n_tail; i += 64u) {
+        uint32_t c = i + (i >= head_lo ? head_n : 0u);
+        if (head2_n) c += c >= head2_lo ? head2_n : 0u;
+        stream_store_rt(dst + c, srcv[c], wt);
+    }
+}
+
 template <bool WT>
 __device__ __forceinline__ void stream_row_dyn(uint4* __restrict__ dst, const uint4* srcv, const uint16_t* tab, uint32_t n_dyn, uint32_t c0, uint32_t c1,
                                                uint32_t lane) {
@@ -258,13 +278,25 @@
     }
 }
 
-template <bool WT>
-__device__ __forceinline__ void store_heads(int8_t* __restrict__ obs, uint64_t obs_stride, int64_t env0, int64_t n_here, uint32_t head_lo,
-                                            uint32_t head_n, const uint4& v, uint32_t lane, uint32_t rot = 0, uint32_t head2_lo = 0, uint32_t head2_n = 0) {
+enum HeadPath { HP_NONE = 0, HP_HOT = 1, HP_COLD = 2 };
+
+__device__ __forceinline__ void store_heads_hot(int8_t* __restrict__ obs, uint32_t obs_stride, int64_t env0, uint32_t n_rows, uint32_t head_lo, uint32_t head_n,
+                                                const uint4& v, uint32_t lane, uint32_t head2_lo, uint32_t head2_n) {
     const uint32_t chunk = lane < head_n ? head_lo + lane : head2_lo + (lane - head_n);
-    if (lane < head_n + head2_n)
-        for (uint32_t k = 0; k < (uint32_t)n_here; k++)
-            stream_store<WT>(reinterpret_cast<uint4*>(obs + (uint64_t)(env0 + rotated(k, rot, (uint32_t)n_here)) * obs_stride) + chunk, v);
+    if (lane < head_n + head2_n) {
+        uint8_t* p = reinterpret_cast<uint8_t*>(obs) + (uint64_t)env0 * obs_stride + (uint64_t)chunk * 16u;
+#pragma clang loop unroll(disable)
+        for (uint32_t k = 0; k < n_rows; k++, p += obs_stride) stream_store<true>(reinterpret_cast<uint4*>(p), v);
+    }
+}
+__device__ __forceinline__ void store_heads_cold(int8_t* __restrict__ obs, uint64_t obs_stride, int64_t env0, uint32_t n_rows, uint32_t head_lo, uint32_t head_n,
+                                                 const uint4& v, uint32_t lane, uint32_t rot, uint32_t head2_lo, uint32_t head2_n, uint32_t wt) {
+    const uint32_t chunk = lane < head_n ? head_lo + lane : head2_lo + (lane - head_n);
+    if (lane < head_n + head2_n) {
+#pragma clang loop unroll(disable)
+        for (uint32_t k = 0; k < n_rows; k++)
+            stream_store_rt(reinterpret_cast<uint4*>(obs + (uint64_t)(env0 + rotated(k, rot, n_rows)) * obs_stride) + chunk, v, wt);
+    }
 }
 
 template <bool CAN_WIDE, typename F>
@@ -281,13 +313,16 @@
     else f(std::false_type{}, std::false_type{});
 }
 
-template <bool WT, bool HEAD = false, bool INCR = false, bool WIDE = false>
+template <bool WT, bool HEAD = false, bool INCR = false, bool WIDE = false, int HP = HP_NONE>
 __device__ __forceinline__ void write_observations(int A, int L, uint32_t D, uint32_t n_chunks, uint64_t obs_stride,
                                                    const uint64_t* dyn, int8_t* tmpl, const uint32_t* scratch,
                                                    uint32_t scr_stride, int8_t* __restrict__ obs, int64_t env0,
                                                    int64_t n_here, uint32_t lane, uint32_t head_lo = 0, uint32_t head_n = 0, uint32_t rot = 0,
-                                                   const uint16_t* dyn_chunks = nullptr, uint32_t n_dyn_chunks = 0, uint32_t et = OBS_I8) {
+                                                   const uint16_t* dyn_chunks = nullptr, uint32_t n_dyn_chunks = 0, uint32_t et = OBS_I8, uint32_t wt_rt = 0) {
     static_assert(!(WIDE && HEAD), "the kernels with row heads carry no widening code: the launcher never sends them a widened launch");
+    static_assert(HP == HP_NONE || (HEAD && !INCR && !WIDE && (HP == HP_COLD || WT)), "the hot path is the write-through tail stream");
+    const uint32_t n_rows = HP != HP_NONE ? (uint32_t)__builtin_amdgcn_readfirstlane((int)n_here) : (uint32_t)n_here;
+    if (HP == HP_HOT) rot = 0u;
     uint32_t dc0 = 0xFFFFu, dc1 = 0xFFFFu;
     if constexpr (INCR) {
         dc0 = lane < n_dyn_chunks ? (uint32_t)dyn_chunks[lane] : 0xFFFFu;
@@ -305,8 +340,8 @@
     const bool is_agent_lane = (int)lane < A;
     const uint4* srcv = reinterpret_cast<const uint4*>(tmpl);
 
-    for (uint32_t k0 = 0; k0 < (uint32_t)n_here; k0++) {
-        const uint32_t k = rotated(k0, rot, (uint32_t)n_here);
+    for (uint32_t k0 = 0; k0 < n_rows; k0++) {
+        const uint32_t k = HP == HP_HOT ? k0 : rotated(k0, rot, n_rows);
         const uint32_t* sc = scratch + k * scr_stride;
         {
             const uint32_t lit = ((sc[d0_w0] >> d0_s0) | (sc[d0_w1] >> d0_s1) | (sc[d0_wg] >> d0_sg)) & 1u;
@@ -330,6 +365,7 @@
             if constexpr (INCR) stream_wide_dyn<WT>(dst, tmpl, dyn_chunks, 0u, n_dyn_chunks, 0u, et, lane);
             else stream_wide<WT>(dst, tmpl, n_chunks, et, lane);
         } else if constexpr (INCR) stream_row_dyn<WT>(dst, srcv, dyn_chunks, n_dyn_chunks, dc0, dc1, lane);
+        else if constexpr (HP == HP_COLD) stream_row_tail_rt(dst, srcv, n_chunks, head_lo, head_n, lane, wt_rt);
         else if constexpr (HEAD) stream_row_tail<WT>(dst, srcv, n_chunks, head_lo, head_n, lane);
         else stream_whole_row<WT>(dst, srcv, n_chunks, lane);
         wave_sync();
@@ -418,7 +454,7 @@
     val = type == ELEM_SOURCE ? -1 : 1;
     on = type == ELEM_SOURCE ? true : (is_gem ? ((sc[L + 1] >> i5) & 1u) != 0 : ((sc[1 + i5] >> off) & 1u) != 0);
 }
-template <bool WT, bool HEAD = false, bool INCR = false, bool WIDE = false>
+template <bool WT, bool HEAD = false, bool INCR = false, bool WIDE = false, int HP = HP_NONE>
 __device__ __forceinline__ void write_observations_env(int A, int L, uint32_t HW, uint32_t n_elems, uint32_t n_chunks,
                                                        uint64_t obs_stride, const uint32_t* elems, const int8_t* bare,
                                                        int8_t* tmpl, const uint32_t* scratch, uint32_t scr_stride,
@@ -426,8 +462,11 @@
                                                        const uint8_t* laser_layer = nullptr, uint32_t gem_layer_in = 0xFFFFFFFFu,
                                                        uint32_t head_lo = 0, uint32_t head_n = 0, uint32_t rot = 0,
                                                        const uint16_t* dyn_chunks = nullptr, uint32_t n_dyn_chunks = 0, uint32_t head2_lo = 0, uint32_t head2_n = 0,
-                                                       uint32_t et = OBS_I8) {
+                                                       uint32_t et = OBS_I8, uint32_t wt_rt = 0) {
     static_assert(!(WIDE && HEAD), "no widening in the kernels with row heads");
+    static_assert(HP == HP_NONE || (HEAD && !INCR && !WIDE && (HP == HP_COLD || WT)), "the hot path is the write-through tail stream");
+    const uint32_t n_rows = HP != HP_NONE ? (uint32_t)__builtin_amdgcn_readfirstlane((int)n_here) : (uint32_t)n_here;
+    if (HP == HP_HOT) rot = 0u;
     uint32_t dc0 = 0xFFFFu, dc1 = 0xFFFFu;
     if constexpr (INCR) {
         dc0 = lane < n_dyn_chunks ? (uint32_t)dyn_chunks[lane] : 0xFFFFu;
@@ -446,8 +485,8 @@
     const uint32_t e0_always = (has_e0 && e0_src) ? 1u : 0u, e0_dyn = (has_e0 && !e0_src) ? 1u : 0u;
     const bool is_agent_lane = (int)lane < A;
     const uint4* srcv = reinterpret_cast<const uint4*>(tmpl);
-    for (uint32_t k0 = 0; k0 < (uint32_t)n_here; k0++) {
-        const uint32_t k = rotated(k0, rot, (uint32_t)n_here);
+    for (uint32_t k0 = 0; k0 < n_rows; k0++) {
+        const uint32_t k = HP == HP_HOT ? k0 : rotated(k0, rot, n_rows);
         const uint32_t* sc = scratch + k * scr_stride;
         const uint32_t colour = (sc[e0_colw] >> e0_colsh) & 0xFFu, onw = sc[e0_onw];
         uint32_t idx0 = e0_base + __umul24(colour, e0_mul);
@@ -467,6 +506,7 @@
             if constexpr (INCR) stream_wide_dyn<WT>(dst, tmpl, dyn_chunks, 0u, n_dyn_chunks, 0u, et, lane);
             else stream_wide<WT>(dst, tmpl, n_chunks, et, lane);
         } else if constexpr (INCR) stream_row_dyn<WT>(dst, srcv, dyn_chunks, n_dyn_chunks, dc0, dc1, lane);
+        else if constexpr (HP == HP_COLD) stream_row_tail_rt(dst, srcv, n_chunks, head_lo, head_n, lane, wt_rt, head2_lo, head2_n);
         else if constexpr (HEAD) stream_row_tail<WT>(dst, srcv, n_chunks, head_lo, head_n, lane, head2_lo, head2_n);
         else stream_whole_row<WT>(dst, srcv, n_chunks, lane);
         wave_sync();
diff --git a/lle_amd/csrc/step_kernel.hpp b/lle_amd/csrc/step_kernel.hpp
--- a/lle_amd/csrc/step_kernel.hpp
+++ b/lle_amd/csrc/step_kernel.hpp
@@ -20,6 +20,13 @@
 __device__ __forceinline__ const EnvOutputs* kernarg_env_out() {
     return reinterpret_cast<const EnvOutputs*>((const char*)__builtin_amdgcn_kernarg_segment_ptr() + KERNARG_ENV_OUT);
 }
+
+__device__ __forceinline__ uint32_t park_uniform(uint32_t s) {
+    uint32_t v;
+    asm("v_mov_b32 %0, %1" : "=v"(v) : "s"(s));
+    return v;
+}
+__device__ __forceinline__ uint32_t unpark_uniform(uint32_t v) { return (uint32_t)__builtin_amdgcn_readfirstlane((int)v); }
 
 template <int G, int LM, int MODE, bool ML1, int LX = -1>
 __global__ void __launch_bounds__(256, (G >= 8 ? 3 : 4)) step_kernel(BatchPtrs P, LaunchArgs K) {
@@ -45,7 +52,8 @@
     const uint32_t EPW = K.envs_per_wave < (uint32_t)(64 / G) ? K.envs_per_wave : (uint32_t)(64 / G);
     constexpr int NW = (2 * G + 7) / 8;
     extern __shared__ __attribute__((aligned(16))) uint8_t lds[];
-    const uint32_t lane = threadIdx.x & 63u, wave_in_wg = threadIdx.x >> 6, waves_per_wg = blockDim.x >> 6;
+    const uint32_t lane = threadIdx.x & 63u, waves_per_wg = blockDim.x >> 6;
+    const uint32_t wave_in_wg = HEAD ? (uint32_t)__builtin_amdgcn_readfirstlane((int)(threadIdx.x >> 6)) : threadIdx.x >> 6;
     const uint32_t blk = xcd_block_dir(blockIdx.x, gridDim.x, K.flags);
     const uint32_t wave_id = blk * waves_per_wg + wave_in_wg;
     const uint8_t* __restrict__ tables = P.tables;
@@ -91,7 +99,11 @@
     uint32_t h_init_beams[LR];
 #pragma unroll
     for (int b = 0; b < LR; b++) h_init_beams[b] = (!BM && b < L) ? initp->beams[b] : 0u;
-    const int64_t n_here = (K.env_limit - env0) < (int64_t)EPW ? (K.env_limit - env0) : (int64_t)EPW;
+    const int64_t n_left = K.env_limit - env0;
+    const int64_t n_here = HEAD ? (int64_t)(n_left < 0 ? 0u : (n_left < (int64_t)EPW ? (uint32_t)n_left : EPW)) : (n_left < (int64_t)EPW ? n_left : (int64_t)EPW);
+    const uint32_t n_rows = n_here > 0 ? (uint32_t)n_here : 0u;
+    constexpr uint32_t HOT_RULES = LAUNCH_WRITE_THROUGH | LAUNCH_ROTATE_ROWS | (MODE == 6 ? LAUNCH_HEAD_GROUP2 | LAUNCH_HEAD_GROUP4 : 0u);
+    const bool hot = HEAD && (K.flags & HOT_RULES) == LAUNCH_WRITE_THROUGH;
     const uint32_t amask = (1u << A) - 1u;
 #define LLE_ROT() ((ROLL && PES) ? 0u : row_rotation(wave_id, EPW, n_here, K.flags))
     LLE_STAMP(0);
@@ -175,11 +187,24 @@
         } \
     } while (0)
 
-    const uint32_t head_lo = HEAD ? (PES ? hdr->pes_head_lo : hdr->head_lo) : 0u;
-    const uint32_t head_n = (HEAD && write_obs && !split && !incr) ? (PES ? hdr->pes_head_n : hdr->head_n) : 0u;
-    const uint32_t head2_lo = (HEAD && PES) ? hdr->pes_head2_lo : 0u, head2_n = (HEAD && PES && head_n) ? hdr->pes_head2_n : 0u;
+    uint32_t head_lo = HEAD ? (PES ? hdr->pes_head_lo : hdr->head_lo) : 0u;
+    const uint32_t head_n_map = HEAD ? (PES ? hdr->pes_head_n : hdr->head_n) : 0u, head2_n_map = (HEAD && PES) ? hdr->pes_head2_n : 0u;
+    const uint32_t head_n = (HEAD && write_obs && !split && !incr) ? head_n_map : 0u;
+    const uint32_t head2_lo = (HEAD && PES) ? hdr->pes_head2_lo : 0u, head2_n = (HEAD && PES && head_n) ? head2_n_map : 0u;
     uint4 head_v = {0u, 0u, 0u, 0u};
     if (HEAD) {
+        const uint32_t q_lay = hdr->off_cell_lay, q_lds = hdr->lds_table_bytes, q_ig = initp->gems;
+        const uint64_t q_ib = initp->bits;
+        asm("" : "+s"(head_lo) : "s"(h_HW), "s"(h_obs_stride), "s"(h_n_chunks), "s"(h_D), "s"(h_enabled), "s"(h_off_cell_meta), "s"(h_off_dyn), "s"(h_off_template),
+                                 "s"(head_n_map), "s"(q_lay), "s"(q_lds), "s"(q_ig), "s"((uint32_t)q_ib), "s"((uint32_t)(q_ib >> 32)), "s"(A), "s"(W),
+                                 "s"((uint32_t)hdr->obs_supported));
+#pragma unroll
+        for (int b = 0; b < LR; b++)
+            if (!BM && b < L) asm("" : "+s"(head_lo) : "s"(h_beam_full[b]), "s"(h_init_beams[b]));
+        if (BM) asm("" : "+s"(head_lo) : "s"(h_chain));
+        if (PES) asm("" : "+s"(head_lo) : "s"(h_off_recolour), "s"(h_off_bare), "s"(h_off_elems), "s"(h_n_elems), "s"(head2_lo), "s"(head2_n_map), "s"((uint32_t)hdr->ext_bytes),
+                                          "s"((uint32_t)hdr->recolour_exact));
+        if (ENV_OUT) asm("" : "+s"(head_lo) : "s"(h_G), "s"(h_H));
         if (lane < head_n + head2_n)
             head_v = reinterpret_cast<const uint4*>(tables + (PES ? h_off_bare : h_off_template))[lane < head_n ? head_lo + lane : head2_lo + (lane - head_n)];
         LLE_LOAD_STATE();
@@ -211,12 +236,12 @@
         if (lane < TMPL_NEG_MAX) pre_neg = reinterpret_cast<const uint32_t*>(tables + sizeof(MapHeader) + tmpl_bits_bytes(h_n_chunks))[lane];
         if (!HEAD) LLE_LOAD_STATE();
     }
-    if (PES) copy_tables2_to_lds(tables + tab_off, tab_bytes, tables + h_off_bare, ext_bytes, lds, lane, wave_in_wg, waves_per_wg);
+    if (PES) copy_tables2_to_lds<HEAD>(tables + tab_off, tab_bytes, tables + h_off_bare, ext_bytes, lds, lane, wave_in_wg, waves_per_wg);
     else if (use_sets) copy_tables2_to_lds(tables + tab_off, tab_bytes, K.win_sets + (uint64_t)map_idx * win_table_bytes(hdr->HW), ext_bytes, lds, lane, wave_in_wg, waves_per_wg);
     else if (CAN_SPLIT && GEN && split && (K.flags & LAUNCH_PACKED_TABLES))
         expand_packed_tables(tables + hdr->off_packed, lds, h_HW, hdr->packed_n_lay, h_off_cell_meta - tab_off, h_off_dyn - tab_off, h_off_template - h_off_dyn,
                              threadIdx.x, blockDim.x);
-    else copy_tables_to_lds(tables + tab_off, lds, tab_bytes, lane, wave_in_wg, waves_per_wg);
+    else copy_tables_to_lds<HEAD>(tables + tab_off, lds, tab_bytes, lane, wave_in_wg, waves_per_wg);
     constexpr uint32_t bt_bytes = BM ? 2u * LM * 4u : 0u;
     uint32_t* beam_tab = reinterpret_cast<uint32_t*>(lds + tab_bytes + ext_bytes);
     if (BM && (int)threadIdx.x < L) {
@@ -234,11 +259,12 @@
     if (HEAD) {
         __builtin_amdgcn_s_waitcnt(0x0F70);
         const uint32_t hgroup = MODE != 6 ? 1u : ((K.flags & LAUNCH_HEAD_GROUP4) ? 4u : ((K.flags & LAUNCH_HEAD_GROUP2) ? 2u : 1u));
-        if (hgroup == 1u) {
-            if (head_n && n_here > 0) {
-                if (K.flags & LAUNCH_WRITE_THROUGH) store_heads<true>(P.obs, h_obs_stride, env0, n_here, head_lo, head_n, head_v, lane, LLE_ROT(), head2_lo, head2_n);
-                else store_heads<false>(P.obs, h_obs_stride, env0, n_here, head_lo, head_n, head_v, lane, LLE_ROT(), head2_lo, head2_n);
-            }
+        const uint32_t wt = K.flags & LAUNCH_WRITE_THROUGH;
+        if (__builtin_expect(hot, 1)) {
+            if (head_n && n_rows) store_heads_hot(P.obs, h_obs_stride, env0, n_rows, head_lo, head_n, head_v, lane, head2_lo, head2_n);
+            asm volatile("s_waitcnt lgkmcnt(0)\n\ts_barrier" ::: "memory");
+        } else if (hgroup == 1u) {
+            if (head_n && n_rows) store_heads_cold(P.obs, h_obs_stride, env0, n_rows, head_lo, head_n, head_v, lane, LLE_ROT(), head2_lo, head2_n, wt);
             asm volatile("s_waitcnt lgkmcnt(0)\n\ts_barrier" ::: "memory");
         } else {
             asm volatile("s_waitcnt lgkmcnt(0)\n\ts_barrier" ::: "memory");
@@ -247,10 +273,7 @@
                     const int64_t e0q = env0 + (int64_t)q * EPW;
                     int64_t nq = K.env_limit - e0q;
                     nq = nq < 0 ? 0 : (nq > (int64_t)EPW ? (int64_t)EPW : nq);
-                    if (nq > 0) {
-                        if (K.flags & LAUNCH_WRITE_THROUGH) store_heads<true>(P.obs, h_obs_stride, e0q, nq, head_lo, head_n, head_v, lane);
-                        else store_heads<false>(P.obs, h_obs_stride, e0q, nq, head_lo, head_n, head_v, lane);
-                    }
+                    if (nq > 0) store_heads_cold(P.obs, h_obs_stride, e0q, (uint32_t)nq, head_lo, head_n, head_v, lane, 0u, 0u, 0u, wt);
                 }
             }
         }
@@ -259,6 +282,8 @@
         if (!(CAN_SPLIT && split)) LLE_LOAD_STATE();
     }
 
+    const uint32_t pk_wave = HEAD ? park_uniform(wave_id) : 0u, pk_env_lo = HEAD ? park_uniform((uint32_t)env0) : 0u,
+                   pk_env_hi = HEAD ? park_uniform((uint32_t)((uint64_t)env0 >> 32)) : 0u;
     const uint64_t* cell_lay = reinterpret_cast<const uint64_t*>(lds);
     const uint32_t* cell_meta = reinterpret_cast<const uint32_t*>(lds + (h_off_cell_meta - tab_off));
     const uint64_t* dyn = reinterpret_cast<const uint64_t*>(lds + (h_off_dyn - tab_off));
@@ -422,6 +447,9 @@
                                                alive, arrived, occ, gems, beams, err, evw, n_ev, meta_step, stepped, nullptr, bm, beam_tab, h_chain);
     LLE_STAMP(3);
 
+    const uint32_t wave_id_l = HEAD ? unpark_uniform(pk_wave) : wave_id;
+    const int64_t env0_l = HEAD ? (int64_t)(((uint64_t)unpark_uniform(pk_env_hi) << 32) | unpark_uniform(pk_env_lo)) : env0;
+#define LLE_ROT_L() ((ROLL && PES) ? 0u : row_rotation(wave_id_l, EPW, n_here, K.flags))
     auto post_step = [&]() {
     LLE_ENV_LATE(env_p);
     if (stepped) avail_lanes<G>(a, me, pos, occ, alive, arrived, meta_step, avail);
@@ -495,7 +523,7 @@
                 if (staged) {
                     wave_sync();
                     const float4* src4 = reinterpret_cast<const float4*>(reinterpret_cast<uint8_t*>(scratch) + st_off);
-                    float4* dst4 = reinterpret_cast<float4*>(O.state + env0 * len);
+                    float4* dst4 = reinterpret_cast<float4*>(O.state + env0_l * len);
                     const uint32_t n4 = n_here > 0 ? (uint32_t)n_here * (uint32_t)len / 4u : 0u;
                     for (uint32_t c = lane; c < n4; c += 64u) dst4[c] = src4[c];
                     wave_sync();
@@ -578,22 +606,41 @@
         const EnvOutputs O = load_uniform(kernarg_env_out());
         if (O.partial && n_here > 0)
             write_partial<true>(A, L, W, (int)K.partial_k, part_pitch, K.partial_E, h_max_layers, cell_lay, cell_meta, part_bm, part_col, tmpl, scratch,
-                                scr_stride, O.partial, env0, n_here, lane, use_sets ? reinterpret_cast<const uint64_t*>(lds + tab_bytes) : nullptr, et);
-    } else if (write_obs && n_here > 0) {
+                                scr_stride, O.partial, env0_l, n_here, lane, use_sets ? reinterpret_cast<const uint64_t*>(lds + tab_bytes) : nullptr, et);
+    } else if (HEAD && write_obs && n_here > 0) {
+        uint32_t lflags = K.flags;
+        asm volatile("" : "+s"(lflags));
+        if (__builtin_expect((lflags & HOT_RULES) == LAUNCH_WRITE_THROUGH, 1)) {
+            if (PES)
+                write_observations_env<true, true, false, false, HP_HOT>(A, L, h_HW, h_n_elems, h_n_chunks, LLE_PITCH(), elems, bare, tmpl, scratch, scr_stride, obs_out, env0_l, n_here,
+                                                                         lane, nullptr, 0xFFFFFFFFu, head_lo, head_n, 0u, nullptr, 0u, head2_lo, head2_n, et);
+            else
+                write_observations<true, true, false, false, HP_HOT>(A, L, h_D, h_n_chunks, LLE_PITCH(), dyn, tmpl, scratch, scr_stride, obs_out, env0_l, n_here, lane, head_lo, head_n,
+                                                                     0u, nullptr, 0u, et);
+        } else {
+            if (PES)
+                write_observations_env<false, true, false, false, HP_COLD>(A, L, h_HW, h_n_elems, h_n_chunks, LLE_PITCH(), elems, bare, tmpl, scratch, scr_stride, obs_out, env0_l, n_here,
+                                                                           lane, nullptr, 0xFFFFFFFFu, head_lo, head_n, LLE_ROT_L(), nullptr, 0u, head2_lo, head2_n, et,
+                                                                           K.flags & LAUNCH_WRITE_THROUGH);
+            else
+                write_observations<false, true, false, false, HP_COLD>(A, L, h_D, h_n_chunks, LLE_PITCH(), dyn, tmpl, scratch, scr_stride, obs_out, env0_l, n_here, lane, head_lo, head_n,
+                                                                       LLE_ROT_L(), nullptr, 0u, et, K.flags & LAUNCH_WRITE_THROUGH);
+        }
+    } else if (!HEAD && write_obs && n_here > 0) {
         dispatch_stream<!HEAD>(K.flags, [&](auto wt_, auto wide_) {
             constexpr bool WT = decltype(wt_)::value, WIDE = decltype(wide_)::value;
             if (PES && CAN_INCR && incr)
-                write_observations_env<WT, false, true, WIDE>(A, L, h_HW, h_n_elems, h_n_chunks, LLE_PITCH(), elems, bare, tmpl, scratch, scr_stride, obs_out, env0, n_here,
-                                                              lane, nullptr, 0xFFFFFFFFu, 0u, 0u, LLE_ROT(), dyn_chunks, h_n_dyn_chunks, 0u, 0u, et);
+                write_observations_env<WT, false, true, WIDE>(A, L, h_HW, h_n_elems, h_n_chunks, LLE_PITCH(), elems, bare, tmpl, scratch, scr_stride, obs_out, env0_l, n_here,
+                                                              lane, nullptr, 0xFFFFFFFFu, 0u, 0u, LLE_ROT_L(), dyn_chunks, h_n_dyn_chunks, 0u, 0u, et);
             else if (PES)
-                write_observations_env<WT, HEAD, false, WIDE>(A, L, h_HW, h_n_elems, h_n_chunks, LLE_PITCH(), elems, bare, tmpl, scratch, scr_stride, obs_out, env0, n_here,
-                                                              lane, nullptr, 0xFFFFFFFFu, head_lo, head_n, LLE_ROT(), nullptr, 0u, head2_lo, head2_n, et);
+                write_observations_env<WT, HEAD, false, WIDE>(A, L, h_HW, h_n_elems, h_n_chunks, LLE_PITCH(), elems, bare, tmpl, scratch, scr_stride, obs_out, env0_l, n_here,
+                                                              lane, nullptr, 0xFFFFFFFFu, head_lo, head_n, LLE_ROT_L(), nullptr, 0u, head2_lo, head2_n, et);
             else if (CAN_INCR && incr)
-                write_observations<WT, false, true, WIDE>(A, L, h_D, h_n_chunks, LLE_PITCH(), dyn, tmpl, scratch, scr_stride, obs_out, env0, n_here, lane, 0u, 0u, LLE_ROT(),
+                write_observations<WT, false, true, WIDE>(A, L, h_D, h_n_chunks, LLE_PITCH(), dyn, tmpl, scratch, scr_stride, obs_out, env0_l, n_here, lane, 0u, 0u, LLE_ROT_L(),
                                                           dyn_chunks, h_n_dyn_chunks, et);
             else
-                write_observations<WT, HEAD, false, WIDE>(A, L, h_D, h_n_chunks, LLE_PITCH(), dyn, tmpl, scratch, scr_stride, obs_out, env0, n_here, lane, head_lo, head_n,
-                                                          LLE_ROT(), nullptr, 0u, et);
+                write_observations<WT, HEAD, false, WIDE>(A, L, h_D, h_n_chunks, LLE_PITCH(), dyn, tmpl, scratch, scr_stride, obs_out, env0_l, n_here, lane, head_lo, head_n,
+                                                          LLE_ROT_L(), nullptr, 0u, et);
         });
     }
     wave_sync();
@@ -621,6 +668,7 @@
 #undef LLE_ENV_LATE
 #undef LLE_LOAD_STATE
 #undef LLE_ROT
+#undef LLE_ROT_L
 #undef LLE_ET
 #undef LLE_PITCH
     }
@@ -628,7 +676,7 @@
         cnt.steps = cnt_lds[0]; cnt.gems = cnt_lds[1]; cnt.exits = cnt_lds[2]; cnt.died = cnt_lds[3];
         cnt.invalid = cnt_lds[4]; cnt.resets = cnt_lds[5]; cnt.bonus = cnt_lds[6];
     }
-    flush_stats(P.stats, wave_id, cnt, A, lane, PRE_STATS, stats_old);
+    flush_stats(P.stats, HEAD ? unpark_uniform(pk_wave) : wave_id, cnt, A, lane, PRE_STATS, stats_old);
     if (STAMPED && stamps) {
         asm volatile("s_waitcnt vmcnt(0)" ::: "memory");
         LLE_STAMP(6);
```

New measurement: 13.58 billion (median of 6 runs). 1.03x the previous value.
